# hihixuyang/LQR-Obstacles

Measured on AMD Instinct MI355X. Metric: agent-pair LQR-obstacle evals/sec, higher is better.
Workload: dtype f64

## Files before the change

### lqr-obstacles_amd/csrc/lqro_qhull3.hpp

```cpp
#pragma once
#include "lqro_qhull.hpp"
#include "lqro_lp.hpp"

namespace lqro {

#ifndef Q3_NEWCAP
#define Q3_NEWCAP 128
#endif
#ifndef Q3_VISCAP
#define Q3_VISCAP 192
#endif
#define Q3_MOVCAP 16
#define Q3_HZCAP 24
#define Q3_COPCAP 8
#define Q3_FSTK 512
#define Q3_ND (Q3_NEWCAP + Q3_MOVCAP)
#define Q3_WAVES 4
#define Q3_HR 4
#ifndef Q3_W0_SLEEP
#define Q3_W0_SLEEP 1
#endif
#ifndef Q3_W1_SLEEP
#define Q3_W1_SLEEP 1
#endif
#ifndef Q3_W2_SLEEP
#define Q3_W2_SLEEP 1
#endif
#ifndef Q3_FL
#define Q3_FL 2240
#endif
#define Q3_PROF_RETRY (32 + 2 * 4096 + 16)
#ifdef LQRO_QHULL_PROFILE
#define Q3_CAPBIT(b) (b)
#else
#define Q3_CAPBIT(b) 0
#endif

struct Q3G {
  double pl[4];
  int nb[3];
  int fa;
  unsigned key;
  unsigned cc;
  int pad[2];
};

struct Q3V {
  double p[9];
  double pad;
  int id[4];
};

struct Q3W {
  double* Pr;
  double* Pf;
  Q3G* G;
  Q3V* vv;
  double* ncoord;
  int* soff;
  double* fdist;
  int* sb;
  int* pq;
  int* pdst;
  double* pdd;
  double* ncoord2;
  unsigned* mark2;
  unsigned* ctr;
  unsigned short* hvis;
  int* hcop;
  int* fq;
  unsigned* fqk;
  HullPt* fqc;
  int FC, SB, HNP, QC;
};

__host__ __device__ inline size_t q3_align(size_t b) { return (b + 255) & ~(size_t)255; }

__host__ __device__ inline size_t q3_worker_bytes(int HNP) {
  const size_t FC = 2 * (size_t)HNP + Q3_NEWCAP + 16, SB = (size_t)QH_SBMULT * HNP, QC = 4 * (size_t)HNP + 64;
  const size_t NG = FC > Q3_FL ? FC - Q3_FL : 1;
  return q3_align(24 * (size_t)HNP) * 2 + q3_align(64 * NG) + q3_align(96 * FC) + q3_align(72 * Q3_NEWCAP) +
         q3_align(4 * FC) +
         q3_align(8 * FC) + q3_align(4 * SB) + q3_align(4 * (size_t)HNP) * 2 + q3_align(8 * (size_t)HNP) +
         q3_align(4 * QC) * 2 + q3_align(32 * QC) + q3_align(72 * Q3_NEWCAP) + q3_align(4 * FC) + 256 +
         q3_align(2 * (Q3_WAVES - 1) * Q3_HZCAP * 64) + q3_align(4 * (Q3_WAVES - 1) * Q3_COPCAP * 64);
}

__device__ inline Q3W q3_worker(char* base, int HNP) {
  Q3W W;
  W.HNP = HNP;
  W.FC = 2 * HNP + Q3_NEWCAP + 16;
  W.SB = QH_SBMULT * HNP;
  W.QC = 4 * HNP + 64;
  const size_t NG = W.FC > Q3_FL ? W.FC - Q3_FL : 1;
  char* p = base;
  auto take = [&](size_t bytes) { char* r = p; p += q3_align(bytes); return r; };
  W.Pr = reinterpret_cast<double*>(take(24 * (size_t)HNP));
  W.Pf = reinterpret_cast<double*>(take(24 * (size_t)HNP));
  W.G = reinterpret_cast<Q3G*>(take(64 * NG));
  W.vv = reinterpret_cast<Q3V*>(take(96 * (size_t)W.FC));
  W.ncoord = reinterpret_cast<double*>(take(72 * (size_t)Q3_NEWCAP));
  W.soff = reinterpret_cast<int*>(take(4 * (size_t)W.FC));
  W.fdist = reinterpret_cast<double*>(take(8 * (size_t)W.FC));
  W.sb = reinterpret_cast<int*>(take(4 * (size_t)W.SB));
  W.pq = reinterpret_cast<int*>(take(4 * (size_t)HNP));
  W.pdst = reinterpret_cast<int*>(take(4 * (size_t)HNP));
  W.pdd = reinterpret_cast<double*>(take(8 * (size_t)HNP));
  W.fq = reinterpret_cast<int*>(take(4 * (size_t)W.QC));
  W.fqk = reinterpret_cast<unsigned*>(take(4 * (size_t)W.QC));
  W.fqc = reinterpret_cast<HullPt*>(take(32 * (size_t)W.QC));
  W.ncoord2 = reinterpret_cast<double*>(take(72 * (size_t)Q3_NEWCAP));
  W.mark2 = reinterpret_cast<unsigned*>(take(4 * (size_t)W.FC));
  W.ctr = reinterpret_cast<unsigned*>(take(256));
  W.hvis = reinterpret_cast<unsigned short*>(take(2 * (Q3_WAVES - 1) * Q3_HZCAP * 64));
  W.hcop = reinterpret_cast<int*>(take(4 * (Q3_WAVES - 1) * Q3_COPCAP * 64));
  return W;
}

struct Q3L {
  int n, fail, job, slot;
  double eps;
  double tr[3 * 128];
  double rk[4];
  int ri[4];
  int scan[4];
  double4 pl[Q3_FL];
  ushort4 tp[Q3_FL];
  unsigned key[Q3_FL];
  unsigned cc[Q3_FL];
  unsigned short fstk[Q3_FSTK];
  int visf[Q3_VISCAP];
  int vsoff[Q3_VISCAP], vscnt[Q3_VISCAP], vinc[Q3_VISCAP];
  int vvert[3 * Q3_VISCAP];
  int repl[Q3_VISCAP];
  int nslot[Q3_NEWCAP];
  int nv[3 * Q3_NEWCAP];
  int nhz[Q3_NEWCAP], nhskip[Q3_NEWCAP];
  int nn1[Q3_NEWCAP], nn2[Q3_NEWCAP];
  alignas(32) double npl[4 * Q3_NEWCAP];
  int nflag[Q3_NEWCAP];
  int movf[Q3_MOVCAP];
  int oldf[Q3_MOVCAP];
  int dfac[Q3_ND], dcnt[Q3_ND], doff[Q3_ND], dchamp[Q3_ND], pcnt[Q3_ND];
  double dmax[Q3_ND];
  double dchp[3 * Q3_ND];
  int cop[Q3_COPCAP * 64];
  unsigned short hvis[Q3_HZCAP * 64];
  int sp_visf[Q3_VISCAP];
  int sp_repl[Q3_VISCAP];
  int sp_v1[Q3_NEWCAP], sp_v2[Q3_NEWCAP], sp_nhz[Q3_NEWCAP], sp_nhskip[Q3_NEWCAP], sp_nflag[Q3_NEWCAP];
  int sp_nn1[Q3_NEWCAP], sp_nn2[Q3_NEWCAP];
  int sp_vvert[3 * Q3_VISCAP];
  alignas(32) double sp_npl[4 * Q3_NEWCAP];
  unsigned short mark[Q3_FL];
  unsigned short sp_cand[3 * Q3_VISCAP];
  int sp_hz, sp_hnvis, pf_done, pf_np;
  int pf_vsoff[Q3_VISCAP], pf_vscnt[Q3_VISCAP];
  HullPt pf_pre[64];
  unsigned char pf_prea[64];
  double sp_apex[3];
  double c_dist[8];
  double c_interior[3];
  int ph, sp_done, sp_ok, sp_facet, sp_furthest, sp_pos, sp_nvis, sp_nnew, sp_status, sp_sharp;
  int sp_gdone;
  unsigned sp_key;
  int pub_qhead, pub_qtail;
  int pub_adopt, pub_nnew;
  double hr_d[Q3_HR * 64];
  unsigned short hr_f[Q3_HR * 64];
  unsigned short hr_k[Q3_HR * 64];
  int hr_ls[Q3_HR], hr_st[Q3_HR];
  unsigned hctl;
  int hbusy, hcons;
  unsigned ectl;
  int edone, ej_np, ej_nd, ej_ndnew, ej_init, ej_nvis;
  int hq_end, hq_from, hq_np, hq_sharp, hq_init;
  int hq_findbestnew, hq_notsharp, hq_nnew, hq_nmov, hq_nvis;
  double hq_max_outside;
#ifdef LQRO_QHULL_LONGPROF
  unsigned long long hprof[12];
  unsigned long long lp_pubr, lp_doner;
#endif
  int big_slot;
  int qflags;
#ifdef LQRO_QHULL_PROFILE
  unsigned long long pub_t, done_t, done_t2;
  unsigned long long pub_r, start_r, done_r;
#endif
};
static_assert(sizeof(Q3L) <= 160 * 1024, "k_qhull's LDS exceeds a CU");

struct Q3S {
  int nalloc, nfs, sbtop, status, qhead, qtail;
  int nins;
  unsigned keyc;
  unsigned key0_last;
  int nnew, nvis, nmov, nold;
  int findbestnew, notsharp;
  int hgen;
  int egen;
  double MAXabs_coord, MAXsumcoord, MAXwidth, NEARzero[3];
  double DISTround, MINvisible, MAXcoplanar, MINoutside, MINdenom, MINdenom_2, max_outside;
  double interior[3];
  unsigned long long tph[32];
  unsigned long long tq;
  unsigned long long tw, nw;
  unsigned long long tdl;
  unsigned long long tw1, nw1;
  unsigned long long tse, tsn;
  unsigned long long tfr, nsp;
  unsigned long long tfr2, trel;
  unsigned long long r_start, r_done, r_seen, r_gseen;
  unsigned long long tseen, tpre, npre, tstart;
  int prev1;
  unsigned long long tps[24], nps;
  unsigned long long lp_n, lp_pts, lp_t, lp_all, lp_tloc, lp_wait, lp_adopt, lp_tail, lp_tw;
  unsigned long long lp_own, lp_got, lp_hwait, lp_stop, lp_ev, lp_posts;
};

#if defined(LQRO_QHULL_PROFILE) && defined(LQRO_QHULL_PROF_LIGHT)
#define Q3T(k) do { const unsigned long long t_ = __builtin_amdgcn_s_memtime(); S.tph[k] += t_ - S.tq; S.tq = t_; } while (0)
#elif defined(LQRO_QHULL_PROFILE)
#define Q3T(k) do { __builtin_amdgcn_s_waitcnt(0); const unsigned long long t_ = __builtin_amdgcn_s_memtime(); S.tph[k] += t_ - S.tq; S.tq = t_; } while (0)
#else
#define Q3T(k) do {} while (0)
#endif
#define Q3_PROF_W1 (32 + 2 * 4096 + 48 + 4 * 4096)
#define Q3_PROF_LONG (Q3_PROF_W1 + 64)
struct Q3P {
  unsigned long long tq2 = 0;
  unsigned long long t[16];
  unsigned long long tq;
};
#if defined(LQRO_QHULL_PROFILE) && defined(LQRO_QHULL_PROF_LIGHT)
#define W1T(k) do { const unsigned long long t_ = __builtin_amdgcn_s_memtime(); P.t[k] += t_ - P.tq; P.tq = t_; } while (0)
#elif defined(LQRO_QHULL_PROFILE)
#define W1T(k) do { __builtin_amdgcn_s_waitcnt(0); const unsigned long long t_ = __builtin_amdgcn_s_memtime(); P.t[k] += t_ - P.tq; P.tq = t_; } while (0)
#else
#define W1T(k) do {} while (0)
#endif
#ifdef LQRO_QHULL_PROFILE
#define Q3C(k, v) do { S.tph[k] += (unsigned long long)(v); } while (0)
#else
#define Q3C(k, v) do {} while (0)
#endif

#define Q3_AS3 __attribute__((address_space(3)))
#define Q3_AS1 __attribute__((address_space(1)))
template <class T> __device__ __forceinline__ T q3_lds(const T& r) { return *(const Q3_AS3 T*)(&r); }
template <class T> __device__ __forceinline__ void q3_lds_st(T& r, const T& v) { *(Q3_AS3 T*)(&r) = v; }
template <class T> __device__ __forceinline__ T q3_glb(const T& r) { return *(const Q3_AS1 T*)(&r); }
template <class T> __device__ __forceinline__ void q3_glb_st(T& r, const T& v) { *(Q3_AS1 T*)(&r) = v; }
typedef double q3_v4d __attribute__((ext_vector_type(4)));
typedef int q3_v4i __attribute__((ext_vector_type(4)));
typedef unsigned q3_v2u __attribute__((ext_vector_type(2)));
__device__ __forceinline__ double4 q3_lds(const double4& r) {
  const q3_v4d v = *(const Q3_AS3 q3_v4d*)(&r);
  return make_double4(v.x, v.y, v.z, v.w);
}
__device__ __forceinline__ void q3_lds_st(double4& r, const double4& v) {
  q3_v4d t; t.x = v.x; t.y = v.y; t.z = v.z; t.w = v.w;
  *(Q3_AS3 q3_v4d*)(&r) = t;
}
__device__ __forceinline__ ushort4 q3_lds(const ushort4& r) {
  const q3_v2u v = *(const Q3_AS3 q3_v2u*)(&r);
  return make_ushort4((unsigned short)(v.x & 0xffffu), (unsigned short)(v.x >> 16), (unsigned short)(v.y & 0xffffu),
                      (unsigned short)(v.y >> 16));
}
__device__ __forceinline__ void q3_lds_st(ushort4& r, const ushort4& v) {
  q3_v2u t;
  t.x = (unsigned)v.x | ((unsigned)v.y << 16);
  t.y = (unsigned)v.z | ((unsigned)v.w << 16);
  *(Q3_AS3 q3_v2u*)(&r) = t;
}
__device__ __forceinline__ double4 q3_glb(const double4& r) {
  const q3_v4d v = *(const Q3_AS1 q3_v4d*)(&r);
  return make_double4(v.x, v.y, v.z, v.w);
}
__device__ __forceinline__ void q3_glb_st(double4& r, const double4& v) {
  q3_v4d t; t.x = v.x; t.y = v.y; t.z = v.z; t.w = v.w;
  *(Q3_AS1 q3_v4d*)(&r) = t;
}
__device__ __forceinline__ int4 q3_glb(const int4& r) {
  const q3_v4i v = *(const Q3_AS1 q3_v4i*)(&r);
  return make_int4(v.x, v.y, v.z, v.w);
}
__device__ __forceinline__ void q3_glb_st(int4& r, const int4& v) {
  q3_v4i t; t.x = v.x; t.y = v.y; t.z = v.z; t.w = v.w;
  *(Q3_AS1 q3_v4i*)(&r) = t;
}

struct Q3Col {
  unsigned short* vis;
  int* cop;
};
template <bool G, class T> __device__ __forceinline__ T q3_col(const T& r) {
  if constexpr (G) return q3_glb(r);
  else return q3_lds(r);
}
template <bool G, class T> __device__ __forceinline__ void q3_col_st(T& r, const T& v) {
  if constexpr (G) q3_glb_st(r, v);
  else q3_lds_st(r, v);
}
__device__ __forceinline__ Q3Col q3_col0(const Q3L& L, int lane) {
  Q3Col C;
  C.vis = const_cast<unsigned short*>(L.hvis) + lane;
  C.cop = const_cast<int*>(L.cop) + lane;
  return C;
}
__device__ __forceinline__ Q3Col q3_colh(const Q3W& W, int wave, int lane) {
  Q3Col C;
  C.vis = W.hvis + (size_t)(wave - 1) * Q3_HZCAP * 64 + lane;
  C.cop = W.hcop + (size_t)(wave - 1) * Q3_COPCAP * 64 + lane;
  return C;
}

__device__ __forceinline__ void q3_get(const Q3W& W, const Q3L& L, int f, double* q, int* nb, int* fa) {
  if (f < Q3_FL) {
    const double4 p = q3_lds(L.pl[f]);
    const ushort4 t = q3_lds(L.tp[f]);
    q[0] = p.x; q[1] = p.y; q[2] = p.z; q[3] = p.w;
    nb[0] = t.x; nb[1] = t.y; nb[2] = t.z; *fa = t.w;
  } else {
    const Q3G& g = W.G[f - Q3_FL];
    const double4 p = q3_glb(*reinterpret_cast<const double4*>(g.pl));
    const int4 t = q3_glb(*reinterpret_cast<const int4*>(g.nb));
    q[0] = p.x; q[1] = p.y; q[2] = p.z; q[3] = p.w;
    nb[0] = t.x; nb[1] = t.y; nb[2] = t.z; *fa = t.w;
  }
}
__device__ __forceinline__ void q3_pl(const Q3W& W, const Q3L& L, int f, double* q) {
  const double4 p = f < Q3_FL ? q3_lds(L.pl[f]) : q3_glb(*reinterpret_cast<const double4*>(W.G[f - Q3_FL].pl));
  q[0] = p.x; q[1] = p.y; q[2] = p.z; q[3] = p.w;
}
__device__ __forceinline__ int q3_nb(const Q3W& W, const Q3L& L, int f, int k) {
  if (f < Q3_FL) return q3_lds(reinterpret_cast<const unsigned short*>(&L.tp[f])[k]);
  return q3_glb(W.G[f - Q3_FL].nb[k]);
}
__device__ __forceinline__ void q3_tp(const Q3W& W, const Q3L& L, int f, int* nb, int* fa) {
  if (f < Q3_FL) {
    const ushort4 t = q3_lds(L.tp[f]);
    nb[0] = t.x; nb[1] = t.y; nb[2] = t.z; *fa = t.w;
  } else {
    const int4 t = q3_glb(*reinterpret_cast<const int4*>(W.G[f - Q3_FL].nb));
    nb[0] = t.x; nb[1] = t.y; nb[2] = t.z; *fa = t.w;
  }
}
__device__ __forceinline__ int q3_fa(const Q3W& W, const Q3L& L, int f) {
  return f < Q3_FL ? (int)q3_lds(L.tp[f].w) : q3_glb(W.G[f - Q3_FL].fa);
}
__device__ __forceinline__ unsigned q3_key(const Q3W& W, const Q3L& L, int f) {
  return f < Q3_FL ? q3_lds(L.key[f]) : q3_glb(W.G[f - Q3_FL].key);
}
__device__ __forceinline__ unsigned q3_cc(const Q3W& W, const Q3L& L, int f) {
  return f < Q3_FL ? q3_lds(L.cc[f]) : q3_glb(W.G[f - Q3_FL].cc);
}
__device__ __forceinline__ void q3_set_fa(const Q3W& W, Q3L& L, int f, int fa) {
  if (f < Q3_FL) q3_lds_st(L.tp[f].w, (unsigned short)fa);
  else q3_glb_st(W.G[f - Q3_FL].fa, fa);
}
__device__ __forceinline__ void q3_set_nb(const Q3W& W, Q3L& L, int f, int k, int v) {
  if (f < Q3_FL) q3_lds_st(reinterpret_cast<unsigned short*>(&L.tp[f])[k], (unsigned short)v);
  else q3_glb_st(W.G[f - Q3_FL].nb[k], v);
}
__device__ __forceinline__ void q3_set_key(const Q3W& W, Q3L& L, int f, unsigned k) {
  if (f < Q3_FL) q3_lds_st(L.key[f], k);
  else q3_glb_st(W.G[f - Q3_FL].key, k);
}
__device__ __forceinline__ void q3_set_cc(const Q3W& W, Q3L& L, int f, unsigned c) {
  if (f < Q3_FL) q3_lds_st(L.cc[f], c);
  else q3_glb_st(W.G[f - Q3_FL].cc, c);
}
__device__ __forceinline__ void q3_set_facet(const Q3W& W, Q3L& L, int f, const double* q, int nb0, int nb1, int nb2,
                                             int fa) {
  if (f < Q3_FL) {
    q3_lds_st(L.pl[f], make_double4(q[0], q[1], q[2], q[3]));
    q3_lds_st(L.tp[f], make_ushort4((unsigned short)nb0, (unsigned short)nb1, (unsigned short)nb2, (unsigned short)fa));
  } else {
    Q3G& g = W.G[f - Q3_FL];
    q3_glb_st(*reinterpret_cast<double4*>(g.pl), make_double4(q[0], q[1], q[2], q[3]));
    q3_glb_st(*reinterpret_cast<int4*>(g.nb), make_int4(nb0, nb1, nb2, fa));
  }
}

__device__ __forceinline__ QhS q3_as_qhs(const Q3S& S) {
  QhS T;
  T.DISTround = S.DISTround;
  T.MINdenom = S.MINdenom;
  T.MINdenom_2 = S.MINdenom_2;
  for (int k = 0; k < 3; k++) T.NEARzero[k] = S.NEARzero[k];
  return T;
}

__device__ inline void q3_plane(const Q3S& S, int& status, const double* r0, const double* r1, const double* r2,
                                int top, double* q, bool* flipped) {
  const double dX10 = r1[0] - r0[0], dY10 = r1[1] - r0[1], dZ10 = r1[2] - r0[2];
  const double dX20 = r2[0] - r0[0], dY20 = r2[1] - r0[1], dZ20 = r2[2] - r0[2];
  double n[3];
  n[0] = QH_DET2(dY20, dZ20, dY10, dZ10);
  n[1] = QH_DET2(dX10, dZ10, dX20, dZ20);
  n[2] = QH_DET2(dX20, dY20, dX10, dY10);
  double norm = sqrt(n[0] * n[0] + n[1] * n[1] + n[2] * n[2]);
  if (norm > S.MINdenom) {
    if (!top) norm = -norm;
    n[0] /= norm;
    n[1] /= norm;
    n[2] /= norm;
  } else {
    status |= QHS_SINGULAR;
  }
  double off = -(r0[0] * n[0] + r0[1] * n[1] + r0[2] * n[2]);
  const double d2 = off + (r2[0] * n[0] + r2[1] * n[1] + r2[2] * n[2]);
  const double d1 = off + (r1[0] * n[0] + r1[1] * n[1] + r1[2] * n[2]);
  if (d2 > S.DISTround || d2 < -S.DISTround || d1 > S.DISTround || d1 < -S.DISTround) {
    const QhS T = q3_as_qhs(S);
    qh_plane_gauss(T, status, r0, r1, r2, top, n, &off);
  }
  q[0] = n[0]; q[1] = n[1]; q[2] = n[2]; q[3] = off;
  const double di = off + S.interior[0] * n[0] + S.interior[1] * n[1] + S.interior[2] * n[2];
  *flipped = di >= -S.DISTround;
}

__device__ __forceinline__ double q3_distq(const double* q, const double* p) {
  return q[3] + p[0] * q[0] + p[1] * q[1] + p[2] * q[2];
}

__device__ __forceinline__ int q3_scan_add(int v) {
  v += __builtin_amdgcn_update_dpp(0, v, 0x111, 0xf, 0xf, false);
  v += __builtin_amdgcn_update_dpp(0, v, 0x112, 0xf, 0xf, false);
  v += __builtin_amdgcn_update_dpp(0, v, 0x114, 0xf, 0xf, false);
  v += __builtin_amdgcn_update_dpp(0, v, 0x118, 0xf, 0xf, false);
  v += __builtin_amdgcn_update_dpp(0, v, 0x142, 0xa, 0xf, false);
  v += __builtin_amdgcn_update_dpp(0, v, 0x143, 0xc, 0xf, false);
  return v;
}

#define Q3_MAXSTEP(V, CTRL, RM)                                                                    \
  do {                                                                                           \
    const long long u_ = __double_as_longlong(V);                                                \
    const int lo_ = __builtin_amdgcn_update_dpp(-1, (int)u_, CTRL, RM, 0xf, false);              \
    const int hi_ = __builtin_amdgcn_update_dpp((int)0xFFEFFFFF, (int)(u_ >> 32), CTRL, RM, 0xf, false); \
    V = fmax(V, __longlong_as_double(((long long)hi_ << 32) | (long long)(unsigned)lo_));        \
  } while (0)
__device__ __forceinline__ double q3_scan_max(double v) {
  Q3_MAXSTEP(v, 0x111, 0xf);
  Q3_MAXSTEP(v, 0x112, 0xf);
  Q3_MAXSTEP(v, 0x114, 0xf);
  Q3_MAXSTEP(v, 0x118, 0xf);
  Q3_MAXSTEP(v, 0x142, 0xa);
  Q3_MAXSTEP(v, 0x143, 0xc);
  return v;
}

__device__ __forceinline__ void q3_place(unsigned long long grp, int lane, unsigned long long ltmask,
                                         double dd, const HullPt& pt, int off, int lim, int& cnt, double& mx,
                                         int& champ, double& cx, double& cy, double& cz, int& wpos, int& wr) {
  const bool mem = (grp >> lane) & 1ull;
  const int cb = cnt + __popcll(grp & ltmask);
  double run = -DBL_MAX;
  if (grp & (grp - 1ull)) {
    const double inc = q3_scan_max(mem ? dd : -DBL_MAX);
    const long long u_ = __double_as_longlong(inc);
    const int lo_ = __builtin_amdgcn_update_dpp(-1, (int)u_, 0x138, 0xf, 0xf, false);
    const int hi_ = __builtin_amdgcn_update_dpp((int)0xFFEFFFFF, (int)(u_ >> 32), 0x138, 0xf, 0xf, false);
    run = __longlong_as_double(((long long)hi_ << 32) | (long long)(unsigned)lo_);
  }
  if (cnt > 0) run = fmax(run, mx);
  const bool rec = mem && (cb == 0 || run < dd);
  const unsigned long long recm = __ballot(rec);
  const unsigned long long prevm = recm & ltmask;
  int pq = 0;
  if (recm & (recm - 1ull)) {
    const int pl = prevm ? 63 - __clzll((long long)prevm) : lane;
    pq = __shfl(pt.q, pl);
  }
  if (mem && cb > 0 && off + cb - 1 < lim) {
    wpos = off + cb - 1;
    wr = rec ? (prevm ? pq : champ) : pt.q;
  }
  if (recm) {
    const int l = 63 - __clzll((long long)recm);
    champ = __builtin_amdgcn_readlane(pt.q, l);
    cx = hl_rl(pt.x, l); cy = hl_rl(pt.y, l); cz = hl_rl(pt.z, l);
    mx = hl_rl(dd, l);
  }
  cnt += __popcll(grp);
}

template <bool G>
__device__ inline int q3_findbesthorizon(const Q3W& W, const Q3S& S, const Q3L& L, const double* p, int startfacet,
                                         double* bestdist, int& lstatus, const Q3Col& C) {
  int bestfacet = startfacet;
  const double searchdist = S.max_outside + 2 * S.DISTround + fmax(S.MINvisible, S.MAXcoplanar);
  double minsearch = *bestdist - searchdist;
  unsigned short* vis = C.vis;
  int nvis = 0;
  int* cop = C.cop;
  int ncop = 0;
  int nextfacet = -1, nextnb[3] = {-1, -1, -1};
  q3_col_st<G>(vis[0], (unsigned short)startfacet);
  nvis = 1;
  int cur[3] = {q3_nb(W, L, startfacet, 0), q3_nb(W, L, startfacet, 1), q3_nb(W, L, startfacet, 2)};
  for (;;) {
    double q[3][4];
    int fl[3], nn[3][3];
    for (int k = 0; k < 3; k++) q3_get(W, L, cur[k], q[k], nn[k], &fl[k]);
    bool seen3[3] = {false, false, false};
    for (int t = 0; t < nvis; t++) {
      const int v = q3_col<G>(vis[64 * t]);
      seen3[0] |= v == cur[0]; seen3[1] |= v == cur[1]; seen3[2] |= v == cur[2];
    }
    for (int k = 0; k < 3; k++) {
      const int nb = cur[k];
      const bool seen = seen3[k] || (k >= 1 && nb == cur[0]) || (k == 2 && nb == cur[1]);
      if (seen) continue;
      if (nvis == Q3_HZCAP) { lstatus |= QHS_CAPACITY | Q3_CAPBIT(QHS_CAP_HZ); return bestfacet; }
      q3_col_st<G>(vis[64 * nvis], (unsigned short)nb);
      nvis++;
      if (!(fl[k] & QF_FLIPPED)) {
        const double dist = q3_distq(q[k], p);
        if (dist > *bestdist) {
          minsearch = dist - searchdist;
          if (dist > *bestdist + searchdist) ncop = 0;
          bestfacet = nb;
          *bestdist = dist;
        } else if (dist < minsearch) {
          continue;
        }
      }
      if (nextfacet >= 0) {
        if (ncop == Q3_COPCAP) { lstatus |= QHS_CAPACITY | Q3_CAPBIT(QHS_CAP_COP); return bestfacet; }
        q3_col_st<G>(cop[64 * ncop++], nextfacet);
      }
      nextfacet = nb;
      nextnb[0] = nn[k][0]; nextnb[1] = nn[k][1]; nextnb[2] = nn[k][2];
    }
    if (nextfacet >= 0) {
      nextfacet = -1;
      cur[0] = nextnb[0]; cur[1] = nextnb[1]; cur[2] = nextnb[2];
      continue;
    }
    if (!ncop) break;
    int facet;
    if (ncop == 1) { facet = q3_col<G>(cop[0]); ncop = 0; }
    else facet = q3_col<G>(cop[64 * --ncop]);
    cur[0] = q3_nb(W, L, facet, 0); cur[1] = q3_nb(W, L, facet, 1); cur[2] = q3_nb(W, L, facet, 2);
  }
  return bestfacet;
}

template <bool G>
__device__ inline int q3_findbestnew(const Q3W& W, const Q3S& S, const Q3L& L, const double* p, int s0,
                                     double* dist, int bestoutside, int* isoutside, int& lstatus, const Q3Col& C) {
  double bestdist = -DBL_MAX / 2;
  int bestfacet = -1;
  const double distoutside = fmax(2 * S.MINoutside, S.max_outside);
  *isoutside = 1;
  const int total = S.nnew + S.nmov;
  auto fetch = [&](int t, int& f, int& fl, double* q) {
    if (t < S.nnew - s0 || t >= S.nnew - s0 + S.nmov) {
      const int u = t < S.nnew - s0 ? s0 + t : t - (S.nnew - s0) - S.nmov;
      f = L.nslot[u];
      const double4 v = q3_lds(*reinterpret_cast<const double4*>(L.npl + 4 * u));
      q[0] = v.x; q[1] = v.y; q[2] = v.z; q[3] = v.w;
      fl = L.nflag[u];
    } else {
      f = L.movf[t - (S.nnew - s0)];
      q3_pl(W, L, f, q);
      fl = q3_fa(W, L, f);
    }
  };
  for (int t0 = 0; t0 < total; t0 += 4) {
    int f[4], fl[4];
    double q[4][4];
#pragma unroll
    for (int k = 0; k < 4; k++) {
      f[k] = -1; fl[k] = QF_FLIPPED;
      if (t0 + k < total) fetch(t0 + k, f[k], fl[k], q[k]);
    }
#pragma unroll
    for (int k = 0; k < 4; k++) {
      if (fl[k] & QF_FLIPPED) continue;
      const double d = q3_distq(q[k], p);
      if (d > bestdist) {
        bestfacet = f[k];
        if (!bestoutside && d >= distoutside) { *dist = d; return bestfacet; }
        bestdist = d;
      }
    }
  }
  bestfacet = q3_findbesthorizon<G>(W, S, L, p, bestfacet >= 0 ? bestfacet : L.nslot[s0], &bestdist, lstatus, C);
  *dist = bestdist;
  if (bestdist < S.MINoutside) *isoutside = 0;
  return bestfacet;
}

__device__ inline int q3_sharpnewfacets(const Q3S& S, const Q3L& L, int lane) {
  if (S.nnew == 0) return 0;
  const bool q0 = L.npl[0] > 0, q1 = L.npl[1] > 0, q2 = L.npl[2] > 0;
  bool diff = false;
  for (int t = lane; t < S.nnew; t += 64) {
    const double* n = L.npl + 4 * t;
    diff |= (n[0] > 0) != q0 || (n[1] > 0) != q1 || (n[2] > 0) != q2;
  }
  return __ballot(diff) != 0ull;
}

template <bool G>
__device__ inline int q3_locate(const Q3W& W, const Q3S& S, const Q3L& L, const double* p, int s0, int sharp,
                                double* bestdist_out, int* isoutside, int* trigger, int& lstatus, const Q3Col& C) {
  *trigger = 0;
  if (sharp == 2) return q3_findbestnew<G>(W, S, L, p, s0, bestdist_out, 1, isoutside, lstatus, C);
  if (S.findbestnew) return q3_findbestnew<G>(W, S, L, p, s0, bestdist_out, 0, isoutside, lstatus, C);
  double bestdist = -DBL_MAX / 2;
  int bestu = -1;
  *isoutside = 1;
  unsigned long long m0 = 0ull, m1 = 0ull;
  if (!(L.nflag[s0] & QF_FLIPPED)) {
    const double d = q3_distq(L.npl + 4 * s0, p);
    if (d >= S.MINoutside) { *bestdist_out = d; return L.nslot[s0]; }
    bestdist = d;
    bestu = s0;
  }
  if (s0 < 64) m0 |= 1ull << s0; else m1 |= 1ull << (s0 - 64);
  int u = s0;
  while (u >= 0) {
    int nxt = -1;
    const int cand[2] = {L.nn1[u], L.nn2[u]};
    const int cfl[2] = {L.nflag[cand[0]], L.nflag[cand[1]]};
    double cq[2][4];
#pragma unroll
    for (int k = 0; k < 2; k++) {
      const double4 v = q3_lds(*reinterpret_cast<const double4*>(L.npl + 4 * cand[k]));
      cq[k][0] = v.x; cq[k][1] = v.y; cq[k][2] = v.z; cq[k][3] = v.w;
    }
#pragma unroll
    for (int k = 0; k < 2; k++) {
      const int c = cand[k];
      const bool was = c < 64 ? (m0 >> c) & 1ull : (m1 >> (c - 64)) & 1ull;
      if (was) continue;
      if (c < 64) m0 |= 1ull << c; else m1 |= 1ull << (c - 64);
      if (!(cfl[k] & QF_FLIPPED)) {
        const double d = q3_distq(cq[k], p);
        if (d > bestdist) {
          if (d >= S.MINoutside) { *bestdist_out = d; return L.nslot[c]; }
          bestu = c;
          bestdist = d;
          nxt = c;
          break;
        }
      }
    }
    u = nxt;
  }
  if (bestu < 0) return q3_findbestnew<G>(W, S, L, p, 0, bestdist_out, 0, isoutside, lstatus, C);
  if (!S.notsharp && bestdist < -S.DISTround) {
    *trigger = 1;
    if (sharp) return q3_findbestnew<G>(W, S, L, p, bestu, bestdist_out, 0, isoutside, lstatus, C);
  }
  const int bf = q3_findbesthorizon<G>(W, S, L, p, L.nslot[bestu], &bestdist, lstatus, C);
  *bestdist_out = bestdist;
  if (bestdist < S.MINoutside) *isoutside = 0;
  return bf;
}

__device__ __forceinline__ bool q3_in_movf(const Q3S& S, const Q3L& L, int f) {
  for (int t = 0; t < S.nmov; t++)
    if (L.movf[t] == f) return true;
  return false;
}

__device__ __forceinline__ HullPt q3_seqpt(const Q3W& W, const Q3L& L, int nvis, bool init, int pos, int* start) {
  HullPt r;
  if (init) {
    const int q = W.pq[pos];
    r.x = W.Pr[3 * (size_t)q]; r.y = W.Pr[3 * (size_t)q + 1]; r.z = W.Pr[3 * (size_t)q + 2];
    r.q = q;
    r.pad = 0;
    *start = 0;
    return r;
  }
  int a = 0, b = nvis - 1;
  while (a < b) {
    const int mid = (a + b) >> 1;
    if (L.vinc[mid] > pos) b = mid;
    else a = mid + 1;
  }
  *start = L.repl[a] >= 0 ? L.repl[a] : 0;
  const int q = W.sb[L.vsoff[a] + pos - (L.vinc[a] - L.vscnt[a])];
  r.x = W.Pr[3 * (size_t)q]; r.y = W.Pr[3 * (size_t)q + 1]; r.z = W.Pr[3 * (size_t)q + 2];
  r.q = q;
  r.pad = 0;
  return r;
}

__device__ __forceinline__ int q3_ld_acq(const int* p) {
  return __hip_atomic_load(p, __ATOMIC_ACQUIRE, __HIP_MEMORY_SCOPE_WORKGROUP);
}
__device__ __forceinline__ void q3_st_rel(int* p, int v) {
  __hip_atomic_store(p, v, __ATOMIC_RELEASE, __HIP_MEMORY_SCOPE_WORKGROUP);
}
__device__ __forceinline__ void q3_st_rel_lds(int* p, int v) {
  __builtin_amdgcn_fence(__ATOMIC_RELEASE, "workgroup", "local");
  __hip_atomic_store(p, v, __ATOMIC_RELAXED, __HIP_MEMORY_SCOPE_WORKGROUP);
}
__device__ __forceinline__ int q3_wait(const int* p, int v, bool ne) {
  int x = q3_ld_acq(p);
  for (long w = 0; (ne ? x == v : x != v) && w < (1l << 24); ++w) {
    __builtin_amdgcn_s_sleep(Q3_W0_SLEEP);
    x = q3_ld_acq(p);
  }
  return x;
}

template <bool G>
__device__ __forceinline__ void q3_chunk_locate(const Q3W& W, const Q3S& S, const Q3L& L, int c, int from, int np,
                                                int sharp, bool init, int lane, const HullPt& pre, int prestart,
                                                int prec, HullPt& pt, int& f, double& d, int& isout, int& trig,
                                                int& ls, const Q3Col& C) {
  const int pos = c + lane;
  pt = pre;
  f = -1; d = 0.0; isout = 0; trig = 0;
  if (pos >= from && pos < np) {
    int start = prestart;
    if (c != prec) pt = q3_seqpt(W, L, S.nvis, init, pos, &start);
    const double p[3] = {pt.x, pt.y, pt.z};
    f = q3_locate<G>(W, S, L, p, start, sharp, &d, &isout, &trig, ls, C);
  }
}

__device__ inline bool q3_help(const Q3W& W, Q3L& L, int lane, const Q3Col& C) {
  const unsigned v = (unsigned)q3_ld_acq(reinterpret_cast<const int*>(&L.hctl));
  if (v == 0u) return false;
  const int k = (int)(v & 0xffffu);
  if (k >= L.hq_end || k >= hl_ld(&L.hcons) + Q3_HR) return false;
  int got = 0;
  if (lane == 0) {
    __hip_atomic_fetch_add(&L.hbusy, 1, __ATOMIC_SEQ_CST, __HIP_MEMORY_SCOPE_WORKGROUP);
    unsigned e = v;
    got = __hip_atomic_compare_exchange_strong(&L.hctl, &e, v + 1u, __ATOMIC_SEQ_CST, __ATOMIC_SEQ_CST,
                                               __HIP_MEMORY_SCOPE_WORKGROUP);
    if (!got) __hip_atomic_fetch_add(&L.hbusy, -1, __ATOMIC_SEQ_CST, __HIP_MEMORY_SCOPE_WORKGROUP);
  }
  if (!__builtin_amdgcn_readfirstlane(got)) return false;
#ifdef LQRO_QHULL_LONGPROF
  const unsigned long long th0 = __builtin_amdgcn_s_memrealtime();
#endif
  Q3S S;
  S.MINvisible = L.c_dist[0]; S.MAXcoplanar = L.c_dist[1]; S.DISTround = L.c_dist[2];
  S.MINoutside = 2 * S.MINvisible;
  S.findbestnew = L.hq_findbestnew; S.notsharp = L.hq_notsharp;
  S.nnew = L.hq_nnew; S.nmov = L.hq_nmov; S.nvis = L.hq_nvis;
  S.max_outside = L.hq_max_outside;
  HullPt pt, pre;
  pre.x = pre.y = pre.z = 0.0; pre.q = -1; pre.pad = 0;
  int f, isout, trig, ls = 0;
  double d;
  const int from = L.hq_from, np = L.hq_np, pos = 64 * k + lane;
  q3_chunk_locate<true>(W, S, L, 64 * k, from, np, L.hq_sharp, L.hq_init != 0, lane, pre, 0, -1, pt, f, d, isout,
                        trig, ls, C);
#ifdef LQRO_QHULL_LONGPROF
  const unsigned long long th1 = __builtin_amdgcn_s_memrealtime();
#endif
  int kind = 0, dst = -1, dfa = 0;
  if (pos >= from && pos < np) {
    if (isout) {
      dst = f;
      dfa = q3_fa(W, L, f);
      if (!(dfa & QF_NEW) && (q3_cc(W, L, f) & 0xffffu) == 0 && !q3_in_movf(S, L, f)) kind |= 4;
    } else if (d >= -S.MAXcoplanar && d > S.max_outside) {
      kind |= 2;
    }
    if (trig) kind |= 1;
  }
  const bool old = dst >= 0 && !(dfa & QF_NEW);
  const int b = k % Q3_HR;
  L.hr_d[64 * b + lane] = d;
  L.hr_f[64 * b + lane] = (unsigned short)dst;
  L.hr_k[64 * b + lane] = (unsigned short)(kind | (old ? 8 : 0) | ((dst >= 0 && !old ? (dfa >> 8) + 1 : 0) << 8));
  const int st = qh_wave_or(ls);
  if (lane == 0) {
    L.hr_ls[b] = st;
    q3_st_rel_lds(&L.hr_st[b], k + 1);
    __hip_atomic_fetch_add(&L.hbusy, -1, __ATOMIC_SEQ_CST, __HIP_MEMORY_SCOPE_WORKGROUP);
#ifdef LQRO_QHULL_LONGPROF
    const unsigned long long th2 = __builtin_amdgcn_s_memrealtime();
    atomicAdd(&L.hprof[0], 1ull);
    atomicAdd(&L.hprof[1], th1 - th0);
    atomicAdd(&L.hprof[2], th2 - th0);
#endif
  }
  return true;
}

__device__ inline void q3_locate_seq(const Q3W& W, Q3S& S, Q3L& L, int np, int sharp, bool init, int lane,
                                     const HullPt& pre, int prestart, bool havepre, int& rg, double& rd,
                                     HullPt& rpt) {
  for (int t = lane; t < Q3_NEWCAP; t += 64) L.pcnt[t] = 0;
  S.nold = 0;
  rg = -1;
  rd = 0.0;
  rpt = pre;
  hl_sync();
  const bool help = np > 64 && (L.qflags & 1);
  const Q3Col C0 = q3_col0(L, lane);
  auto post = [&](int from2) {
    S.hgen = S.hgen % 32767 + 1;
    if (lane == 0) {
      L.hq_end = (np + 63) >> 6; L.hq_from = from2; L.hq_np = np; L.hq_sharp = sharp; L.hq_init = init ? 1 : 0;
      L.hq_findbestnew = S.findbestnew; L.hq_notsharp = S.notsharp; L.hq_nnew = S.nnew; L.hq_nmov = S.nmov;
      L.hq_nvis = S.nvis; L.hq_max_outside = S.max_outside;
      L.hcons = from2 >> 6;
      for (int b = 0; b < Q3_HR; b++) L.hr_st[b] = 0;
      q3_st_rel(reinterpret_cast<int*>(&L.hctl), (int)(((unsigned)S.hgen << 16) | (unsigned)((from2 >> 6) + 1)));
    }
  };
  auto stop = [&]() {
    if (lane == 0) __hip_atomic_exchange(&L.hctl, 0u, __ATOMIC_SEQ_CST, __HIP_MEMORY_SCOPE_WORKGROUP);
    int b = __hip_atomic_load(&L.hbusy, __ATOMIC_SEQ_CST, __HIP_MEMORY_SCOPE_WORKGROUP);
    for (long w = 0; b != 0 && w < (1l << 24); ++w) {
      __builtin_amdgcn_s_sleep(Q3_W0_SLEEP);
      b = __hip_atomic_load(&L.hbusy, __ATOMIC_SEQ_CST, __HIP_MEMORY_SCOPE_WORKGROUP);
    }
    if (b != 0) S.status |= QHS_CAPACITY | QHS_TIMEOUT;
  };
  int from = 0;
  while (from < np && !(S.status & QHS_CAPACITY)) {
    int ev_pos = np, ev_kind = 0, ev_dst = -1;
    double ev_d = 0.0;
    if (help) post(from);
    bool first = help;
    for (int c = from & ~63; c < np; c += 64) {
      Q3C(23, 1);
      const int pos = c + lane;
      const bool act = pos >= from && pos < np;
      int kind = 0, ls = 0, dst = -1, dfa = 0;
      double d = 0.0;
      HullPt pt = pre;
      int f = -1, isout = 0, trig = 0;
      bool mine = !help || first;
      if (help && !first) {
        const int k = c >> 6, b = k % Q3_HR;
        int st = q3_ld_acq(&L.hr_st[b]);
        if (st != k + 1) {
          int m = 0;
          if (lane == 0) {
            unsigned e = __hip_atomic_load(&L.hctl, __ATOMIC_RELAXED, __HIP_MEMORY_SCOPE_WORKGROUP);
            if ((e & 0xffffu) == (unsigned)k)
              m = __hip_atomic_compare_exchange_strong(&L.hctl, &e, e + 1u, __ATOMIC_RELAXED, __ATOMIC_RELAXED,
                                                       __HIP_MEMORY_SCOPE_WORKGROUP);
          }
          mine = __builtin_amdgcn_readfirstlane(m) != 0;
#ifdef LQRO_QHULL_LONGPROF
          const unsigned long long tw0 = __builtin_amdgcn_s_memrealtime();
#endif
          if (!mine) st = q3_wait(&L.hr_st[b], k + 1, false);
#ifdef LQRO_QHULL_LONGPROF
          if (!mine) S.lp_hwait += __builtin_amdgcn_s_memrealtime() - tw0;
#endif
        }
#ifdef LQRO_QHULL_LONGPROF
        if (mine) S.lp_own++; else S.lp_got++;
#endif
        int kv = 0;
        if (!mine) {
          if (st != k + 1) { S.status |= QHS_CAPACITY | QHS_TIMEOUT; break; }
          const int fv = L.hr_f[64 * b + lane];
          kv = L.hr_k[64 * b + lane];
          ls = L.hr_ls[b];
          dst = fv == 0xffff ? -1 : fv;
          kind = act ? kv & 7 : 0;
          dfa = (kv & 8) ? 0 : (((kv >> 8) - 1) << 8) | QF_NEW;
          d = L.hr_d[64 * b + lane];
        }
      }
      first = false;
      Q3T(12);
      if (mine) q3_chunk_locate<false>(W, S, L, c, from, np, sharp, init, lane, pre, prestart, havepre ? 0 : -1, pt, f,
                                       d, isout, trig, ls, C0);
      Q3T(13);
      if (mine && act) {
        if (isout) {
          dst = f;
          dfa = q3_fa(W, L, f);
          if (!(dfa & QF_NEW) && (q3_cc(W, L, f) & 0xffffu) == 0 && !q3_in_movf(S, L, f)) kind |= 4;
        } else if (d >= -S.MAXcoplanar && d > S.max_outside) {
          kind |= 2;
        }
        if (trig) kind |= 1;
      }
      S.status |= qh_wave_or(ls);
      if (help && lane == 0) q3_st_rel_lds(&L.hcons, (c >> 6) + 1);
      const unsigned long long b = __ballot(kind != 0);
      const int last = b ? __ffsll((long long)b) - 1 : 63;
      const bool fin = act && lane <= last;
      int g = -1;
      if (fin && dst >= 0 && (dfa & QF_NEW)) {
        g = dfa >> 8;
        atomicAdd(&L.pcnt[g], 1);
      }
      unsigned long long old = __ballot(fin && dst >= 0 && !(dfa & QF_NEW));
      while (old) {
        const int l = __ffsll((long long)old) - 1;
        old &= old - 1;
        const int f = __builtin_amdgcn_readlane(dst, l);
        int k = -1;
        for (int t = 0; t < S.nold; t++)
          if (L.oldf[t] == f) k = t;
        if (k < 0) {
          if (S.nold == Q3_MOVCAP) { S.status |= QHS_CAPACITY | Q3_CAPBIT(QHS_CAP_MOV); continue; }
          k = S.nold++;
          if (lane == 0) { L.oldf[k] = f; L.pcnt[Q3_NEWCAP + k] = 0; L.dfac[Q3_NEWCAP + k] = f; }
          hl_sync();
        }
        if (lane == 0) L.pcnt[Q3_NEWCAP + k]++;
        if (lane == l) g = Q3_NEWCAP + k;
        hl_sync();
      }
      if (fin) {
        rg = g;
        rd = d;
        rpt = pt;
        if (np > 64) {
          W.pdst[pos] = g;
          W.pdd[pos] = d;
        }
      }
      hl_sync();
      Q3T(14);
      if (b) {
        ev_pos = c + last;
        ev_kind = __builtin_amdgcn_readlane(kind, last);
        ev_dst = __builtin_amdgcn_readlane(dst, last);
        ev_d = hl_rl(d, last);
        break;
      }
    }
#ifdef LQRO_QHULL_LONGPROF
    const unsigned long long ts0 = __builtin_amdgcn_s_memrealtime();
#endif
    if (help) stop();
#ifdef LQRO_QHULL_LONGPROF
    if (help) { S.lp_stop += __builtin_amdgcn_s_memrealtime() - ts0; S.lp_posts++; if (ev_pos < np) S.lp_ev++; }
#endif
    if (S.status & QHS_CAPACITY) return;
    if (ev_pos < np) {
      Q3C(24, 1);
      if (ev_kind & 1) {
        if (sharp) S.findbestnew = 1;
        else S.notsharp = 1;
      }
      if (ev_kind & 2) S.max_outside = ev_d;
      if (ev_kind & 4) {
        const int f = ev_dst;
        if (S.nmov == Q3_MOVCAP) {
          S.status |= QHS_CAPACITY | Q3_CAPBIT(QHS_CAP_MOV);
          return;
        }
        if (lane == 0) {
          L.movf[S.nmov] = f;
          if (init) {
            int t0 = 0;
            for (int t = 0; t < S.nnew; t++)
              if (L.nslot[t] == f) t0 = t;
            for (int t = t0; t + 1 < S.nnew; t++) {
              L.nslot[t] = L.nslot[t + 1];
              for (int k = 0; k < 4; k++) L.npl[4 * t + k] = L.npl[4 * (t + 1) + k];
              L.nflag[t] = L.nflag[t + 1];
            }
            double q[4];
            q3_pl(W, L, f, q);
            L.nslot[S.nnew - 1] = f;
            for (int k = 0; k < 4; k++) L.npl[4 * (S.nnew - 1) + k] = q[k];
            L.nflag[S.nnew - 1] = q3_fa(W, L, f);
          }
        }
        q3_set_key(W, L, f, S.keyc);
        S.keyc++;
        S.nmov++;
      }
      hl_sync();
    }
    from = ev_pos + 1;
  }
}

__device__ inline void q3_emit_bucket(const Q3W& W, Q3L& L, int lane, int b) {
  const int np = L.ej_np, nd = L.ej_nd, ndnew = L.ej_ndnew, nvis = L.ej_nvis;
  const bool init = L.ej_init != 0;
  const int gl = lane < ndnew ? lane : Q3_NEWCAP + (lane - ndnew);
  const bool has = lane < nd && (lane & 3) == b && L.pcnt[gl];
  int Rc = 0, Rch = -1, Ro = 0;
  double Rm = 0.0, Rx = 0.0, Ry = 0.0, Rz = 0.0;
  if (has) {
    Rc = L.dcnt[gl]; Rm = L.dmax[gl]; Rch = L.dchamp[gl]; Ro = L.doff[gl];
    Rx = L.dchp[3 * gl]; Ry = L.dchp[3 * gl + 1]; Rz = L.dchp[3 * gl + 2];
  }
  const unsigned long long ltmask = (1ull << lane) - 1ull;
  int ng = -1;
  double ndd = 0.0;
  HullPt npt;
  npt.x = npt.y = npt.z = 0.0; npt.q = -1; npt.pad = 0;
  auto ldc = [&](int c) {
    const int pos = c + lane;
    ng = -1;
    ndd = 0.0;
    if (pos < np) {
      ng = W.pdst[pos];
      ndd = W.pdd[pos];
      int st;
      npt = q3_seqpt(W, L, nvis, init, pos, &st);
    }
  };
  ldc(0);
  for (int c = 0; c < np; c += 64) {
    const int g = ng;
    const double dd = ndd;
    const HullPt pt = npt;
    if (c + 64 < np) ldc(c + 64);
    const int i = g < 0 ? -1 : (g < Q3_NEWCAP ? g : ndnew + (g - Q3_NEWCAP));
    const bool mine = i >= 0 && (i & 3) == b;
    unsigned long long todo = __ballot(mine);
    int wpos = -1, wr = 0;
    while (todo) {
      const int lead = __ffsll((long long)todo) - 1;
      const int gg = __builtin_amdgcn_readlane(g, lead);
      const unsigned long long grp = __ballot(mine && g == gg);
      todo &= ~grp;
      const int l = __builtin_amdgcn_readlane(i, lead);
      int cnt = __builtin_amdgcn_readlane(Rc, l), champ = __builtin_amdgcn_readlane(Rch, l);
      double mx = hl_rl(Rm, l), cx = hl_rl(Rx, l), cy = hl_rl(Ry, l), cz = hl_rl(Rz, l);
      q3_place(grp, lane, ltmask, dd, pt, __builtin_amdgcn_readlane(Ro, l), W.SB, cnt, mx, champ, cx, cy, cz, wpos,
               wr);
      if (lane == l) { Rc = cnt; Rm = mx; Rch = champ; Rx = cx; Ry = cy; Rz = cz; }
    }
    if (wpos >= 0) W.sb[wpos] = wr;
  }
  if (has) {
    L.dcnt[gl] = Rc; L.dmax[gl] = Rm; L.dchamp[gl] = Rch;
    L.dchp[3 * gl] = Rx; L.dchp[3 * gl + 1] = Ry; L.dchp[3 * gl + 2] = Rz;
  }
}

__device__ __forceinline__ int q3_emit_claim(Q3L& L, int lane) {
  int k = -1;
  if (lane == 0) {
    for (;;) {
      unsigned v = (unsigned)q3_ld_acq(reinterpret_cast<const int*>(&L.ectl));
      if (v == 0u || (v & 0xffu) >= 4u) break;
      unsigned e = v;
      if (__hip_atomic_compare_exchange_strong(&L.ectl, &e, v + 1u, __ATOMIC_ACQ_REL, __ATOMIC_RELAXED,
                                               __HIP_MEMORY_SCOPE_WORKGROUP)) {
        k = (int)(v & 0xffu);
        break;
      }
    }
  }
  return __builtin_amdgcn_readfirstlane(k);
}

__device__ inline bool q3_emit_help(const Q3W& W, Q3L& L, int lane) {
  const unsigned v = (unsigned)q3_ld_acq(reinterpret_cast<const int*>(&L.ectl));
  if (v == 0u || (v & 0xffu) >= 4u) return false;
  const int k = q3_emit_claim(L, lane);
  if (k < 0) return false;
  q3_emit_bucket(W, L, lane, k);
  if (lane == 0) {
    __builtin_amdgcn_fence(__ATOMIC_RELEASE, "workgroup");
    __hip_atomic_fetch_add(&L.edone, 1, __ATOMIC_RELEASE, __HIP_MEMORY_SCOPE_WORKGROUP);
  }
  return true;
}

__device__ inline void q3_emit_seq(const Q3W& W, Q3S& S, Q3L& L, int np, int ndnew, bool init, int lane, int rg,
                                   double rd, const HullPt& rpt) {
  if (S.status & QHS_CAPACITY) return;
  if (!init && np <= 64 && S.nold == 0 && ndnew <= 64) {
    const int g = lane;
    int pc = 0, f = 0;
    if (g < ndnew) { f = L.nslot[g]; pc = L.pcnt[g]; }
    const int inc = q3_scan_add(pc);
    const int top = S.sbtop + __builtin_amdgcn_readlane(inc, 63);
    if (top > W.SB) {
      S.status |= QHS_CAPACITY | Q3_CAPBIT(QHS_CAP_SB);
      return;
    }
    const int doff = S.sbtop + inc - pc;
    S.sbtop = top;
    Q3T(15);
    int dcnt = 0, dchamp = -1;
    double dmax = 0.0, dx = 0.0, dy = 0.0, dz = 0.0;
    const unsigned long long ltmask = (1ull << lane) - 1ull;
    const int rgl = lane < np ? rg : -1;
    unsigned long long todo = __ballot(rgl >= 0);
    int wpos = -1, wr = 0;
    Q3T(16);
    while (todo) {
      const int lead = __ffsll((long long)todo) - 1;
      const int gg = __builtin_amdgcn_readlane(rgl, lead);
      const unsigned long long grp = __ballot(rgl == gg);
      todo &= ~grp;
      int cnt = 0, champ = -1;
      double mx = 0.0, cx = 0.0, cy = 0.0, cz = 0.0;
      q3_place(grp, lane, ltmask, rd, rpt, __builtin_amdgcn_readlane(doff, gg), W.SB, cnt, mx, champ, cx, cy, cz,
               wpos, wr);
      Q3C(25, 1);
      if (lane == gg) { dcnt = cnt; dmax = mx; dchamp = champ; dx = cx; dy = cy; dz = cz; }
    }
    if (wpos >= 0) W.sb[wpos] = wr;
    Q3T(17);
    if (g < ndnew && pc) {
      W.sb[doff + dcnt - 1] = dchamp;
      W.soff[f] = doff;
      W.fdist[f] = dmax;
      q3_set_cc(W, L, f, (unsigned)dcnt | ((unsigned)dchamp << 16));
    }
    const bool has = g < ndnew && pc > 0;
    const unsigned long long b = __ballot(has);
    int qt = S.qtail;
    if (has) {
      const int at = qt + __popcll(b & ltmask);
      if (at < W.QC) {
        W.fq[at] = f;
        W.fqk[at] = S.key0_last + (unsigned)g;
        HullPt r;
        r.x = dx; r.y = dy; r.z = dz; r.q = dchamp; r.pad = 0;
        W.fqc[at] = r;
      }
    }
    qt += __popcll(b);
    if (qt > W.QC) S.status |= QHS_CAPACITY | Q3_CAPBIT(QHS_CAP_FACETS);
    S.qtail = qt;
    hl_sync();
    Q3T(18);
    return;
  }
  const int nd = ndnew + S.nold;
  int base = S.sbtop;
  for (int c0 = 0; c0 < nd; c0 += 64) {
    const int i = c0 + lane;
    int size = 0, g = -1, cnt0 = 0;
    if (i < nd) {
      g = i < ndnew ? i : Q3_NEWCAP + (i - ndnew);
      if (g < Q3_NEWCAP) L.dfac[g] = L.nslot[g];
      if (L.pcnt[g]) {
        cnt0 = g < Q3_NEWCAP ? 0 : (int)(q3_cc(W, L, L.dfac[g]) & 0xffffu);
        size = cnt0 + L.pcnt[g];
      }
    }
    const int inc = q3_scan_add(size);
    if (size) {
      L.doff[g] = base + inc - size;
      L.dcnt[g] = cnt0;
      L.dmax[g] = 0.0;
      L.dchamp[g] = -1;
    }
    base += __builtin_amdgcn_readlane(inc, 63);
  }
  if (base > W.SB) {
    S.status |= QHS_CAPACITY | Q3_CAPBIT(QHS_CAP_SB);
    return;
  }
  S.sbtop = base;
  hl_sync();
  for (int k = 0; k < S.nold; k++) {
    const int g = Q3_NEWCAP + k;
    const int f = L.dfac[g];
    const int cnt0 = L.dcnt[g];
    if (!L.pcnt[g] || !cnt0) continue;
    const int off0 = W.soff[f];
    const int off = L.doff[g];
    for (int t = lane; t < cnt0 - 1; t += 64) W.sb[off + t] = W.sb[off0 + t];
    const int chq = W.sb[off0 + cnt0 - 1];
    const double fd = W.fdist[f];
    if (lane == 0) {
      L.dchamp[g] = chq;
      L.dchp[3 * g] = W.Pr[3 * (size_t)chq]; L.dchp[3 * g + 1] = W.Pr[3 * (size_t)chq + 1];
      L.dchp[3 * g + 2] = W.Pr[3 * (size_t)chq + 2];
      L.dmax[g] = fd;
    }
    hl_sync();
  }
  hl_sync();
  Q3T(15);
  if (np > 64 && nd <= 64 && (L.qflags & 16)) {
    S.egen = S.egen % 0xffffff + 1;
    if (lane == 0) {
      L.ej_np = np; L.ej_nd = nd; L.ej_ndnew = ndnew; L.ej_init = init ? 1 : 0; L.ej_nvis = S.nvis;
      L.edone = 0;
      q3_st_rel(reinterpret_cast<int*>(&L.ectl), (int)((unsigned)S.egen << 8));
    }
    int mine = 0;
    for (int k = q3_emit_claim(L, lane); k >= 0; k = q3_emit_claim(L, lane)) {
      q3_emit_bucket(W, L, lane, k);
      ++mine;
    }
    hl_sync();
    int dn = q3_ld_acq(&L.edone);
    for (long w = 0; dn != 4 - mine && w < (1l << 24); ++w) {
      __builtin_amdgcn_s_sleep(Q3_W0_SLEEP);
      dn = q3_ld_acq(&L.edone);
    }
    if (lane == 0) __hip_atomic_store(&L.ectl, 0u, __ATOMIC_RELAXED, __HIP_MEMORY_SCOPE_WORKGROUP);
    if (dn != 4 - mine) { S.status |= QHS_CAPACITY | QHS_TIMEOUT; return; }
  } else {
  const bool inl = nd <= 64 && (L.qflags & 2);
  int Rc = 0, Rch = -1, Ro = 0;
  double Rm = 0.0, Rx = 0.0, Ry = 0.0, Rz = 0.0;
  if (inl && lane < nd) {
    const int g = lane < ndnew ? lane : Q3_NEWCAP + (lane - ndnew);
    if (L.pcnt[g]) {
      Rc = L.dcnt[g]; Rm = L.dmax[g]; Rch = L.dchamp[g]; Ro = L.doff[g];
      Rx = L.dchp[3 * g]; Ry = L.dchp[3 * g + 1]; Rz = L.dchp[3 * g + 2];
    }
  }
  int ng = -1;
  double ndd = 0.0;
  HullPt npt = rpt;
  auto ldc = [&](int c) {
    const int pos = c + lane;
    ng = -1;
    ndd = 0.0;
    if (pos < np) {
      ng = W.pdst[pos];
      ndd = W.pdd[pos];
      int st;
      npt = q3_seqpt(W, L, S.nvis, init, pos, &st);
    }
  };
  if (np > 64) ldc(0);
  for (int c = 0; c < np; c += 64) {
    const int pos = c + lane;
    const bool act = pos < np;
    int g = rg;
    double dd = rd;
    HullPt pt = rpt;
    if (np > 64) {
      g = ng;
      dd = ndd;
      pt = npt;
      if (c + 64 < np) ldc(c + 64);
    } else if (!act) {
      g = -1;
    }
    Q3T(16);
    unsigned long long todo = __ballot(g >= 0);
    const unsigned long long ltmask = (1ull << lane) - 1ull;
    int wpos = -1, wr = 0;
    while (todo) {
      const int lead = __ffsll((long long)todo) - 1;
      const int gg = __builtin_amdgcn_readlane(g, lead);
      const unsigned long long grp = __ballot(g == gg);
      todo &= ~grp;
      if (inl) {
        const int l = gg < Q3_NEWCAP ? gg : ndnew + (gg - Q3_NEWCAP);
        int cnt = __builtin_amdgcn_readlane(Rc, l), champ = __builtin_amdgcn_readlane(Rch, l);
        double mx = hl_rl(Rm, l), cx = hl_rl(Rx, l), cy = hl_rl(Ry, l), cz = hl_rl(Rz, l);
        q3_place(grp, lane, ltmask, dd, pt, __builtin_amdgcn_readlane(Ro, l), W.SB, cnt, mx, champ, cx, cy, cz, wpos,
                 wr);
        if (lane == l) { Rc = cnt; Rm = mx; Rch = champ; Rx = cx; Ry = cy; Rz = cz; }
      } else {
        int cnt = L.dcnt[gg];
        double mx = L.dmax[gg];
        int champ = L.dchamp[gg];
        double cx = L.dchp[3 * gg], cy = L.dchp[3 * gg + 1], cz = L.dchp[3 * gg + 2];
        const int off = L.doff[gg];
        q3_place(grp, lane, ltmask, dd, pt, off, W.SB, cnt, mx, champ, cx, cy, cz, wpos, wr);
        if (lane == 0) {
          L.dcnt[gg] = cnt; L.dmax[gg] = mx; L.dchamp[gg] = champ;
          L.dchp[3 * gg] = cx; L.dchp[3 * gg + 1] = cy; L.dchp[3 * gg + 2] = cz;
        }
        hl_sync();
      }
      Q3C(25, 1);
    }
    if (wpos >= 0) W.sb[wpos] = wr;
  }
  if (inl && lane < nd) {
    const int g = lane < ndnew ? lane : Q3_NEWCAP + (lane - ndnew);
    if (L.pcnt[g]) {
      L.dcnt[g] = Rc; L.dmax[g] = Rm; L.dchamp[g] = Rch;
      L.dchp[3 * g] = Rx; L.dchp[3 * g + 1] = Ry; L.dchp[3 * g + 2] = Rz;
    }
  }
  }
  hl_sync();
  Q3T(17);
  for (int i = lane; i < nd; i += 64) {
    const int g = i < ndnew ? i : Q3_NEWCAP + (i - ndnew);
    if (!L.pcnt[g]) continue;
    const int f = L.dfac[g];
    W.sb[L.doff[g] + L.dcnt[g] - 1] = L.dchamp[g];
    W.soff[f] = L.doff[g];
    W.fdist[f] = L.dmax[g];
    q3_set_cc(W, L, f, (unsigned)L.dcnt[g] | ((unsigned)L.dchamp[g] << 16));
  }
  hl_sync();
  if (init) return;
  int qt = S.qtail;
  for (int c = 0; c < ndnew; c += 64) {
    const int t = c + lane;
    const bool has = t < ndnew && L.pcnt[t] > 0;
    const unsigned long long b = __ballot(has);
    if (has) {
      const int at = qt + __popcll(b & ((1ull << lane) - 1ull));
      if (at < W.QC) {
        W.fq[at] = L.nslot[t];
        W.fqk[at] = q3_key(W, L, L.nslot[t]);
        HullPt r;
        r.x = L.dchp[3 * t]; r.y = L.dchp[3 * t + 1]; r.z = L.dchp[3 * t + 2]; r.q = L.dchamp[t]; r.pad = 0;
        W.fqc[at] = r;
      }
    }
    qt += __popcll(b);
  }
  for (int t = lane; t < S.nmov; t += 64)
    if (qt + t < W.QC) {
      W.fq[qt + t] = L.movf[t];
      W.fqk[qt + t] = q3_key(W, L, L.movf[t]);
      HullPt r;
      r.x = r.y = r.z = 0.0; r.q = -1; r.pad = 0;
      W.fqc[qt + t] = r;
    }
  qt += S.nmov;
  if (qt > W.QC) S.status |= QHS_CAPACITY | Q3_CAPBIT(QHS_CAP_FACETS);
  S.qtail = qt;
  hl_sync();
  Q3T(18);
}

__device__ __forceinline__ int q3_alloc(const Q3S& S, const Q3L& L, int t) {
  if (t < S.nvis) return L.visf[t];
  const int e = t - S.nvis;
  if (e < S.nfs) return L.fstk[S.nfs - 1 - e];
  return S.nalloc + (e - S.nfs);
}

struct Q3QC {
  int qcb, qcn, qf, qp;
  unsigned qk;
  double qx, qy, qz;
  int one, rt;
  double r[6];
  int pc_from, pc_pos, pc_end, pc_f, pc_p;
  unsigned pc_k;
  double pc_x, pc_y, pc_z;
};

__device__ inline void q3_spec(const Q3W& W, Q3L& L, int lane, unsigned short ep, unsigned ep2, Q3QC& Q, Q3P& P,
                               int phase) {
  const unsigned long long ltmask = (1ull << lane) - 1ull;
  Q3S C;
  C.MINvisible = L.c_dist[0]; C.MAXcoplanar = L.c_dist[1]; C.DISTround = L.c_dist[2];
  C.MINdenom = L.c_dist[3]; C.MINdenom_2 = L.c_dist[4];
  for (int k = 0; k < 3; k++) { C.NEARzero[k] = L.c_dist[5 + k]; C.interior[k] = L.c_interior[k]; }
  auto marked = [&](int f) -> bool {
    return f < Q3_FL ? q3_lds(L.mark[f]) == ep : q3_glb(W.mark2[f]) == ep2;
  };
  auto mark = [&](int f) {
    if (f < Q3_FL) q3_lds_st(L.mark[f], ep);
    else q3_glb_st(W.mark2[f], ep2);
  };
  if (L.pub_adopt) {
    const int nn = L.pub_nnew;
    if (Q.one) {
      if (Q.rt >= 0) {
        const int t = Q.rt;
        Q3V& v = W.vv[L.nslot[t]];
        *reinterpret_cast<double4*>(v.p) = make_double4(L.sp_apex[0], L.sp_apex[1], L.sp_apex[2], Q.r[0]);
        *reinterpret_cast<double4*>(v.p + 4) = make_double4(Q.r[1], Q.r[2], Q.r[3], Q.r[4]);
        *reinterpret_cast<double2*>(v.p + 8) = make_double2(Q.r[5], 0.0);
        *reinterpret_cast<int4*>(v.id) = make_int4(L.nv[3 * t], L.nv[3 * t + 1], L.nv[3 * t + 2], 0);
      }
    } else {
      for (int t = lane; t < nn; t += 64) {
        Q3V& v = W.vv[L.nslot[t]];
        const double* nc = W.ncoord2 + 9 * t;
        *reinterpret_cast<double4*>(v.p) = make_double4(L.sp_apex[0], L.sp_apex[1], L.sp_apex[2], nc[0]);
        *reinterpret_cast<double4*>(v.p + 4) = make_double4(nc[1], nc[2], nc[3], nc[4]);
        *reinterpret_cast<double2*>(v.p + 8) = make_double2(nc[5], 0.0);
        *reinterpret_cast<int4*>(v.id) = make_int4(L.nv[3 * t], L.nv[3 * t + 1], L.nv[3 * t + 2], 0);
      }
    }
  }
  Q.one = 0;
  Q.rt = -1;
  W1T(1);
#ifdef LQRO_QHULL_LONGPROF
  const unsigned long long tq0_ = __builtin_amdgcn_s_memrealtime();
  int reloads_ = 0;
#endif
  int ok = 0;
  const int qt = L.pub_qtail;
  int facet = -1, furthest = -1, fpos = -1;
  unsigned fkey = 0;
  double apex[3] = {0.0, 0.0, 0.0};
  int qh0 = L.pub_qhead;
  if (Q.pc_from >= 0 && Q.pc_from == qh0 && L.pub_adopt) {
    if (Q.pc_pos >= 0) {
      const int fa = q3_fa(W, L, Q.pc_f);
      const unsigned c = q3_cc(W, L, Q.pc_f);
      if ((fa & QF_LIVE) && !(fa & QF_VISIBLE) && q3_key(W, L, Q.pc_f) == Q.pc_k && (c & 0xffffu) > 0) {
        fpos = Q.pc_pos;
        facet = Q.pc_f;
        fkey = Q.pc_k;
        furthest = (int)(c >> 16);
        if (Q.pc_p == furthest) {
          apex[0] = Q.pc_x; apex[1] = Q.pc_y; apex[2] = Q.pc_z;
        } else {
          apex[0] = W.Pr[3 * (size_t)furthest];
          apex[1] = W.Pr[3 * (size_t)furthest + 1];
          apex[2] = W.Pr[3 * (size_t)furthest + 2];
        }
      } else {
        qh0 = Q.pc_pos + 1;
      }
    } else {
      qh0 = max(qh0, Q.pc_end);
    }
  }
  Q.pc_from = -1;
  for (int qh = qh0; facet < 0 && qh < qt;) {
    if (qh >= Q.qcb + Q.qcn || qh < Q.qcb) {
#ifdef LQRO_QHULL_LONGPROF
      ++reloads_;
#endif
      Q.qcb = qh;
      Q.qcn = min(64, qt - qh);
      if (lane < Q.qcn) {
        Q.qf = W.fq[qh + lane];
        Q.qk = W.fqk[qh + lane];
        const HullPt e = W.fqc[qh + lane];
        Q.qx = e.x; Q.qy = e.y; Q.qz = e.z; Q.qp = e.q;
      }
    }
    bool good = false;
    unsigned c = 0;
    if (lane < Q.qcn && Q.qcb + lane >= qh && Q.qcb + lane < qt) {
      const int fa = q3_fa(W, L, Q.qf);
      c = q3_cc(W, L, Q.qf);
      good = (fa & QF_LIVE) && !(fa & QF_VISIBLE) && q3_key(W, L, Q.qf) == Q.qk && (c & 0xffffu) > 0;
    }
    const unsigned long long b = __ballot(good);
    if (b) {
      const int l = __ffsll((long long)b) - 1;
      fpos = Q.qcb + l;
      facet = __builtin_amdgcn_readlane(Q.qf, l);
      fkey = (unsigned)__builtin_amdgcn_readlane((int)Q.qk, l);
      furthest = (int)((unsigned)__builtin_amdgcn_readlane((int)c, l) >> 16);
      if (__builtin_amdgcn_readlane(Q.qp, l) == furthest) {
        apex[0] = hl_rl(Q.qx, l); apex[1] = hl_rl(Q.qy, l); apex[2] = hl_rl(Q.qz, l);
      } else {
        apex[0] = W.Pr[3 * (size_t)furthest];
        apex[1] = W.Pr[3 * (size_t)furthest + 1];
        apex[2] = W.Pr[3 * (size_t)furthest + 2];
      }
      break;
    }
    qh = Q.qcb + Q.qcn;
  }
  int ls = 0, nvis = 0, nnew = 0, ts = 0, lm = 0;
  W1T(2);
#ifdef LQRO_QHULL_LONGPROF
  const unsigned long long tq1_ = __builtin_amdgcn_s_memrealtime();
  if (lane == 0) { L.hprof[8] += (unsigned long long)reloads_; L.hprof[9] += tq1_ - tq0_; }
#endif
  if (facet >= 0) {
    if (lane == 0) L.sp_visf[0] = facet;
    if (lane < 3) L.sp_cand[lane] = (unsigned short)q3_nb(W, L, facet, lane);
    mark(facet);
    hl_sync();
    nvis = 1;
    bool cap = false;
    for (int lo = 0; lo < nvis && !cap;) {
      const int hi = nvis;
      const int ncand = 3 * (hi - lo);
      for (int c0 = 0; c0 < ncand; c0 += 64) {
        const int c = c0 + lane;
        int nb = -1;
        bool cand = false;
        double q[4] = {0.0, 0.0, 0.0, 0.0};
        int nn[3] = {0, 0, 0};
        if (c < ncand) {
          nb = L.sp_cand[3 * lo + c];
          int fa;
          q3_get(W, L, nb, q, nn, &fa);
          cand = !marked(nb);
        }
        const double dist = cand ? q3_distq(q, apex) : 0.0;
        bool vis = cand && dist >= C.MINvisible;
        if (cand && !vis && dist >= -C.MAXcoplanar) ls |= QHS_COPLANAR;
        bool dup = false;
        for (unsigned long long mm = __ballot(vis); mm;) {
          const int l = __ffsll((long long)mm) - 1;
          mm &= mm - 1;
          dup |= (l < lane) && __builtin_amdgcn_readlane(nb, l) == nb;
        }
        vis = vis && !dup;
        const unsigned long long bv = __ballot(vis);
        if (vis) {
          const int at = nvis + __popcll(bv & ltmask);
          if (at < Q3_VISCAP) {
            L.sp_visf[at] = nb;
            L.sp_cand[3 * at] = (unsigned short)nn[0];
            L.sp_cand[3 * at + 1] = (unsigned short)nn[1];
            L.sp_cand[3 * at + 2] = (unsigned short)nn[2];
          }
          mark(nb);
        }
        nvis += __popcll(bv);
        hl_sync();
      }
      lo = hi;
      if (nvis > Q3_VISCAP) cap = true;
#ifdef LQRO_QHULL_PROFILE
      P.t[11] += 1;
#endif
    }
#ifdef LQRO_QHULL_LONGPROF
    if (lane == 0) L.hprof[10] += __builtin_amdgcn_s_memrealtime() - tq1_;
#endif
    if (!cap && lane == 0) {
      L.sp_hnvis = nvis;
      q3_st_rel_lds(&L.sp_hz, phase);
    }
    W1T(3);
    const bool one = 3 * nvis <= 64;
    int my_t = -1, rv1 = -1, rv2 = -1, mn1 = 0, mn2 = 0;
    double P1[3] = {0.0, 0.0, 0.0}, P2[3] = {0.0, 0.0, 0.0}, PO[3] = {0.0, 0.0, 0.0};
    double Q4[4] = {0.0, 0.0, 0.0, 0.0};
    unsigned long long rb = 0ull;
    if (!cap) {
      for (int vi = lane; vi < nvis; vi += 64) L.sp_repl[vi] = -1;
      hl_sync();
      for (int c0 = 0; c0 < 3 * nvis; c0 += 64) {
        const int c = c0 + lane;
        int vis = -1, nb = -1, hfa = 0;
        bool ridge = false;
        int hn[3] = {-1, -1, -1};
        if (c < 3 * nvis) {
          const int vi = c / 3;
          vis = L.sp_visf[vi];
          nb = L.sp_cand[c];
          q3_tp(W, L, nb, hn, &hfa);
          ridge = !marked(nb);
          if (c == 3 * vi) {
            const Q3V& vw = W.vv[vis];
            L.sp_vvert[3 * vi] = vw.id[0]; L.sp_vvert[3 * vi + 1] = vw.id[1]; L.sp_vvert[3 * vi + 2] = vw.id[2];
          }
        }
        const unsigned long long b = __ballot(ridge);
        if (one) rb = b;
        if (ridge) {
          const int t = nnew + __popcll(b & ltmask);
          const int hskip = hn[0] == vis ? 0 : hn[1] == vis ? 1 : hn[2] == vis ? 2 : -1;
          if (hskip < 0) {
            ts |= QHS_TOPOLOGY;
          } else if (t < Q3_NEWCAP) {
            const Q3V& h = W.vv[nb];
            const int top = (hfa & QF_TOP) ? (hskip & 1) : ((hskip & 1) ^ 1);
            const int i1 = hskip == 0 ? 1 : 0, i2 = hskip == 2 ? 1 : 2;
            double p1[3], p2[3], po[3];
            for (int k = 0; k < 3; k++) {
              p1[k] = h.p[3 * i1 + k];
              p2[k] = h.p[3 * i2 + k];
              po[k] = h.p[3 * hskip + k];
            }
            L.sp_v1[t] = h.id[i1];
            L.sp_v2[t] = h.id[i2];
            L.sp_nhz[t] = nb;
            L.sp_nhskip[t] = hskip;
            atomicMax(&L.sp_repl[c / 3], t);
            double q[4];
            bool flipped;
            int fl = QF_NEW | QF_LIVE | (top ? QF_TOP : 0);
            q3_plane(C, lm, apex, p1, p2, top, q, &flipped);
            if (flipped) { fl |= QF_FLIPPED; lm |= QHS_FLIPPED; }
            L.sp_nflag[t] = fl;
            L.sp_npl[4 * t] = q[0]; L.sp_npl[4 * t + 1] = q[1]; L.sp_npl[4 * t + 2] = q[2]; L.sp_npl[4 * t + 3] = q[3];
            if (one) {
              my_t = t;
              rv1 = h.id[i1];
              rv2 = h.id[i2];
              for (int k = 0; k < 4; k++) Q4[k] = q[k];
              for (int k = 0; k < 3; k++) { P1[k] = p1[k]; P2[k] = p2[k]; PO[k] = po[k]; }
            } else {
              for (int k = 0; k < 3; k++) {
                W.ncoord2[9 * t + k] = p1[k]; W.ncoord2[9 * t + 3 + k] = p2[k]; W.ncoord2[9 * t + 6 + k] = po[k];
              }
            }
          }
        }
        nnew += __popcll(b);
      }
      ok = nnew <= Q3_NEWCAP;
      if (one) {
        Q.one = 1;
        Q.rt = my_t;
        for (int k = 0; k < 3; k++) { Q.r[k] = P1[k]; Q.r[3 + k] = P2[k]; }
      }
      W1T(4);
      if (ok) {
        hl_sync();
        if (one) {
          int nbu[2] = {-1, -1}, cnt[2] = {0, 0};
          int u = 0;
          for (unsigned long long bb = rb; bb; bb &= bb - 1ull, ++u) {
            const int l = __ffsll((long long)bb) - 1;
            const int a = __builtin_amdgcn_readlane(rv1, l), c2 = __builtin_amdgcn_readlane(rv2, l);
            const bool o = u != my_t;
            if (o && (a == rv2 || c2 == rv2)) { nbu[0] = u; cnt[0]++; }
            if (o && (a == rv1 || c2 == rv1)) { nbu[1] = u; cnt[1]++; }
          }
          if (my_t >= 0) {
            if (cnt[0] != 1 || cnt[1] != 1) lm |= QHS_TOPOLOGY;
            mn1 = nbu[0] >= 0 ? nbu[0] : 0;
            mn2 = nbu[1] >= 0 ? nbu[1] : 0;
            L.sp_nn1[my_t] = mn1;
            L.sp_nn2[my_t] = mn2;
          }
        } else {
          for (int t = lane; t < nnew; t += 64) {
            int nbu[2] = {-1, -1}, cnt[2] = {0, 0};
            const int w0 = L.sp_v2[t], w1 = L.sp_v1[t];
#pragma unroll 4
            for (int u = 0; u < nnew; u++) {
              const int a = L.sp_v1[u], bb = L.sp_v2[u];
              const bool o = u != t;
              if (o && (a == w0 || bb == w0)) { nbu[0] = u; cnt[0]++; }
              if (o && (a == w1 || bb == w1)) { nbu[1] = u; cnt[1]++; }
            }
            if (cnt[0] != 1 || cnt[1] != 1) lm |= QHS_TOPOLOGY;
            L.sp_nn1[t] = nbu[0] >= 0 ? nbu[0] : 0;
            L.sp_nn2[t] = nbu[1] >= 0 ? nbu[1] : 0;
          }
        }
        hl_sync();
        W1T(12);
        if (!(qh_wave_or(lm) & QHS_FLIPPED)) {
          auto zero = [&](int t, const double* p1, const double* p2, const double* po) {
            const double d1 = q3_distq(L.sp_npl + 4 * L.sp_nn1[t], p1);
            const double d2 = q3_distq(L.sp_npl + 4 * L.sp_nn2[t], p2);
            const double d3 = q3_distq(L.sp_npl + 4 * t, po);
            if (d1 >= -2 * C.DISTround || d2 >= -2 * C.DISTround || d3 >= -2 * C.DISTround) lm |= QHS_NONCONVEX;
          };
          if (one) {
            if (my_t >= 0) {
              const double4 a = q3_lds(*reinterpret_cast<const double4*>(L.sp_npl + 4 * mn1));
              const double4 b = q3_lds(*reinterpret_cast<const double4*>(L.sp_npl + 4 * mn2));
              const double qa[4] = {a.x, a.y, a.z, a.w}, qb[4] = {b.x, b.y, b.z, b.w};
              const double d1 = q3_distq(qa, P1), d2 = q3_distq(qb, P2), d3 = q3_distq(Q4, PO);
              if (d1 >= -2 * C.DISTround || d2 >= -2 * C.DISTround || d3 >= -2 * C.DISTround) lm |= QHS_NONCONVEX;
            }
          } else {
            for (int t = lane; t < nnew; t += 64) {
              double p1[3], p2[3], po[3];
              for (int k = 0; k < 3; k++) {
                p1[k] = W.ncoord2[9 * t + k]; p2[k] = W.ncoord2[9 * t + 3 + k]; po[k] = W.ncoord2[9 * t + 6 + k];
              }
              zero(t, p1, p2, po);
            }
          }
        }
        W1T(13);
        bool diff = false;
        if (one && rb) {
          const int l0 = __ffsll((long long)rb) - 1;
          const bool q0 = hl_rl(Q4[0], l0) > 0, q1 = hl_rl(Q4[1], l0) > 0, q2 = hl_rl(Q4[2], l0) > 0;
          if (my_t >= 0) diff = (Q4[0] > 0) != q0 || (Q4[1] > 0) != q1 || (Q4[2] > 0) != q2;
        } else if (nnew > 0) {
          const bool q0 = L.sp_npl[0] > 0, q1 = L.sp_npl[1] > 0, q2 = L.sp_npl[2] > 0;
          for (int t = lane; t < nnew; t += 64) {
            const double* nn = L.sp_npl + 4 * t;
            diff |= (nn[0] > 0) != q0 || (nn[1] > 0) != q1 || (nn[2] > 0) != q2;
          }
        }
        const bool sh = __ballot(diff) != 0ull;
        if (lane == 0) L.sp_sharp = sh;
      }
    }
  }
  const int st = qh_wave_or(ls | ts | lm);
  W1T(5);
  hl_sync();
  Q.pc_end = qt;
  if (lane == 0) {
    L.sp_ok = ok;
    L.sp_facet = facet;
    L.sp_key = fkey;
    L.sp_furthest = furthest;
    L.sp_pos = fpos;
    L.sp_nvis = nvis;
    L.sp_nnew = nnew;
    L.sp_status = st;
    L.sp_apex[0] = apex[0]; L.sp_apex[1] = apex[1]; L.sp_apex[2] = apex[2];
  }
}

__device__ inline void q3_prescan(const Q3W& W, Q3L& L, int lane, unsigned short ep, unsigned ep2, Q3QC& Q) {
  Q.pc_from = -1;
  const int from = L.sp_pos, qt = Q.pc_end;
  if (!L.sp_ok || L.sp_facet < 0 || from < 0) return;
  auto marked = [&](int f) -> bool {
    return f < Q3_FL ? q3_lds(L.mark[f]) == ep : q3_glb(W.mark2[f]) == ep2;
  };
  Q.pc_pos = -1;
  for (int qh = from; qh < qt;) {
    if (qh >= Q.qcb + Q.qcn || qh < Q.qcb) {
      Q.qcb = qh;
      Q.qcn = min(64, qt - qh);
      if (lane < Q.qcn) {
        Q.qf = W.fq[qh + lane];
        Q.qk = W.fqk[qh + lane];
        const HullPt e = W.fqc[qh + lane];
        Q.qx = e.x; Q.qy = e.y; Q.qz = e.z; Q.qp = e.q;
      }
    }
    bool good = false;
    if (lane < Q.qcn && Q.qcb + lane >= qh && Q.qcb + lane < qt) {
      const int fa = q3_fa(W, L, Q.qf);
      const unsigned c = q3_cc(W, L, Q.qf);
      good = (fa & QF_LIVE) && !marked(Q.qf) && q3_key(W, L, Q.qf) == Q.qk && (c & 0xffffu) > 0;
    }
    const unsigned long long b = __ballot(good);
    if (b) {
      const int l = __ffsll((long long)b) - 1;
      Q.pc_pos = Q.qcb + l;
      Q.pc_f = __builtin_amdgcn_readlane(Q.qf, l);
      Q.pc_k = (unsigned)__builtin_amdgcn_readlane((int)Q.qk, l);
      Q.pc_p = __builtin_amdgcn_readlane(Q.qp, l);
      Q.pc_x = hl_rl(Q.qx, l); Q.pc_y = hl_rl(Q.qy, l); Q.pc_z = hl_rl(Q.qz, l);
      break;
    }
    qh = Q.qcb + Q.qcn;
  }
  Q.pc_from = from;
}

__device__ inline void q3_prefetch(const Q3W& W, Q3L& L, int lane, int p) {
  const int nvis = L.sp_hnvis;
  int np = 0;
  for (int c0 = 0; c0 < nvis; c0 += 64) {
    const int vi = c0 + lane;
    int cnt = 0;
    if (vi < nvis) {
      const int f = L.sp_visf[vi];
      cnt = (int)(q3_cc(W, L, f) & 0xffffu) - (vi == 0 ? 1 : 0);
      L.pf_vsoff[vi] = W.soff[f];
      L.pf_vscnt[vi] = cnt;
    }
    np += __builtin_amdgcn_readlane(q3_scan_add(cnt), 63);
  }
  hl_sync();
  if (lane < np) {
    int a = 0, base = 0;
    for (;;) {
      const int k = L.pf_vscnt[a];
      if (lane < base + k || a == nvis - 1) break;
      base += k;
      ++a;
    }
    const int q = W.sb[L.pf_vsoff[a] + lane - base];
    HullPt r;
    r.x = W.Pr[3 * (size_t)q]; r.y = W.Pr[3 * (size_t)q + 1]; r.z = W.Pr[3 * (size_t)q + 2];
    r.q = q;
    r.pad = 0;
    L.pf_pre[lane] = r;
    L.pf_prea[lane] = (unsigned char)a;
  }
  hl_sync();
  if (lane == 0) {
    L.pf_np = np;
    q3_st_rel(&L.pf_done, p);
  }
}

__device__ inline void q3_build(const Q3W& W, Q3S& S, Q3L& L, int n, int lane) {
#ifdef LQRO_QHULL_PROFILE
  S.tq = __builtin_amdgcn_s_memtime();
#endif
  const unsigned long long ltmask = (1ull << lane) - 1ull;
  S.status = 0;
  S.nalloc = 1;
  S.nfs = 0;
  S.sbtop = 0;
  S.nnew = S.nvis = S.nmov = S.nold = 0;
  S.findbestnew = S.notsharp = 0;
  S.hgen = 0;
  S.egen = 0;
  S.keyc = 1;
  S.key0_last = 0;
  S.qhead = S.qtail = 0;
  if (W.FC > 65535) {
    S.status |= QHS_CAPACITY | Q3_CAPBIT(QHS_CAP_FACETS);
    return;
  }
  int maxpoints[6];
  S.max_outside = 0.0;
  S.MAXabs_coord = 0.0;
  S.MAXwidth = -DBL_MAX;
  S.MAXsumcoord = 0.0;
  for (int k = 0; k < 3; k++) {
    int mn, mx;
    qh_extreme(W.Pr, n, k, false, lane, &mn);
    qh_extreme(W.Pr, n, k, true, lane, &mx);
    const double maxk = W.Pr[3 * (size_t)mx + k], mink = W.Pr[3 * (size_t)mn + k];
    const double maxcoord = fmax(maxk, -mink);
    const double temp = maxk - mink;
    if (temp > S.MAXwidth) S.MAXwidth = temp;
    if (maxcoord > S.MAXabs_coord) S.MAXabs_coord = maxcoord;
    S.MAXsumcoord += maxcoord;
    maxpoints[2 * k] = mn;
    maxpoints[2 * k + 1] = mx;
    S.NEARzero[k] = 80 * S.MAXsumcoord * DBL_EPSILON;
  }
  {
    double maxdistsum = sqrt(3.0) * S.MAXabs_coord;
    if (S.MAXsumcoord < maxdistsum) maxdistsum = S.MAXsumcoord;
    S.DISTround = DBL_EPSILON * (3 * maxdistsum * 1.01 + S.MAXabs_coord);
    const double MINdenom_1 = fmax(1.0 / DBL_MAX, DBL_MIN);
    S.MINdenom = MINdenom_1 * S.MAXabs_coord;
    S.MINdenom_2 = sqrt(MINdenom_1 * 3) * S.MAXabs_coord;
    S.MINvisible = 0.0 + 2 * S.DISTround;
    S.MAXcoplanar = S.MINvisible;
    S.MINoutside = 2 * S.MINvisible;
  }
  int simplex[4];
  {
    const QhS T = q3_as_qhs(S);
    double maxcoord = -DBL_MAX, mincoord = DBL_MAX;
    int minx = -1, maxx = -1;
    for (int i = 0; i < 6; i++) {
      const double c = W.Pr[3 * (size_t)maxpoints[i]];
      if (maxcoord < c) { maxcoord = c; maxx = maxpoints[i]; }
      if (mincoord > c) { mincoord = c; minx = maxpoints[i]; }
    }
    double maxdet = maxcoord - mincoord;
    int ns = 0;
    simplex[ns++] = minx;
    if (maxx != minx) simplex[ns++] = maxx;
    if (ns < 2) { S.status |= QHS_INPUT; return; }
    for (int i = 2; i < 4; i++) {
      const double prevdet = maxdet;
      int maxpoint = -1, maxnearzero = 0, nearzero;
      maxdet = -1.0;
      for (int m = 0; m < 6; m++) {
        const int p = maxpoints[m];
        bool ins = false;
        for (int t = 0; t < i; t++) ins |= simplex[t] == p;
        if (!ins && p != maxpoint) {
          const double det = fabs(qh_detsimplex(T, W.Pr, simplex, i, p, &nearzero));
          if (det > maxdet) { maxdet = det; maxpoint = p; maxnearzero = nearzero; }
        }
      }
      const double targetdet = prevdet * S.MAXwidth;
      const bool falsenarrow = maxdet > 0.0 && maxdet / targetdet < 1.0e-3;
      if (maxpoint < 0 || maxnearzero || falsenarrow) {
        double key = -1.0;
        int idx = 0x7fffffff;
        for (int q = lane; q < n; q += 64) {
          bool skip = false;
          for (int t = 0; t < 6; t++) skip |= maxpoints[t] == q;
          for (int t = 0; t < i; t++) skip |= simplex[t] == q;
          if (skip) continue;
          const double det = fabs(qh_detsimplex(T, W.Pr, simplex, i, q, &nearzero));
          if (det > key || (det == key && q < idx)) { key = det; idx = q; }
        }
        for (int off = 32; off >= 1; off >>= 1) {
          const double ok = __shfl_xor(key, off);
          const int oi = __shfl_xor(idx, off);
          if (ok > key || (ok == key && oi < idx)) { key = ok; idx = oi; }
        }
        if (idx != 0x7fffffff && key > maxdet) { maxdet = key; maxpoint = idx; }
      }
      if (maxpoint < 0) { S.status |= QHS_INPUT; return; }
      simplex[i] = maxpoint;
    }
  }
  const int pset[4] = {simplex[3], simplex[2], simplex[1], simplex[0]};
  int fs[4];
  {
    int top = 1, tops[4];
    for (int i = 0; i < 4; i++) {
      fs[i] = S.nalloc++;
      tops[i] = top;
      top ^= 1;
    }
    for (int k = 0; k < 3; k++) {
      double c = 0.0;
      for (int t = 0; t < 4; t++) c += W.Pr[3 * (size_t)pset[t] + k];
      S.interior[k] = c / 4;
    }
    int fv[4][3];
    for (int i = 0; i < 4; i++) {
      int m = 0;
      for (int t = 0; t < 4; t++)
        if (t != i) fv[i][m++] = pset[t];
    }
    int ls = 0;
    double q[4][4];
    bool fl[4];
    q3_plane(S, ls, W.Pr + 3 * (size_t)fv[0][0], W.Pr + 3 * (size_t)fv[0][1], W.Pr + 3 * (size_t)fv[0][2], tops[0],
             q[0], &fl[0]);
    if (q3_distq(q[0], S.interior) > S.DISTround)
      for (int i = 0; i < 4; i++) tops[i] ^= 1;
    bool anyflip = false;
    for (int i = 0; i < 4; i++) {
      q3_plane(S, ls, W.Pr + 3 * (size_t)fv[i][0], W.Pr + 3 * (size_t)fv[i][1], W.Pr + 3 * (size_t)fv[i][2],
               tops[i], q[i], &fl[i]);
      anyflip |= fl[i];
    }
    if (anyflip) ls |= QHS_FLIPPED;
    int nbs[4][3];
    for (int i = 0; i < 4; i++) {
      int m = 0;
      for (int t = 0; t < 4; t++)
        if (t != i) nbs[i][m++] = fs[t];
    }
    double minangle = DBL_MAX;
    for (int i = 0; i < 4; i++)
      for (int t = 0; t < 3; t++) {
        int j = 0;
        for (int u = 0; u < 4; u++)
          if (fs[u] == nbs[i][t]) j = u;
        double angle = 0.0;
        for (int k = 0; k < 3; k++) angle += q[i][k] * q[j][k];
        if (angle < minangle) minangle = angle;
      }
    if (minangle < -0.99999999) ls |= QHS_NARROW;
    S.status |= ls;
    hl_sync();
    if (lane == 0)
      for (int i = 0; i < 4; i++) {
        const int f = fs[i];
        q3_set_facet(W, L, f, q[i], nbs[i][0], nbs[i][1], nbs[i][2],
                     QF_LIVE | (tops[i] ? QF_TOP : 0) | (fl[i] ? QF_FLIPPED : 0));
        q3_set_key(W, L, f, S.keyc + i);
        q3_set_cc(W, L, f, 0u);
        Q3V& v = W.vv[f];
        for (int t = 0; t < 3; t++) {
          for (int k = 0; k < 3; k++) v.p[3 * t + k] = W.Pr[3 * (size_t)fv[i][t] + k];
          v.id[t] = fv[i][t];
        }
      }
    S.keyc += 4;
    hl_sync();
    int np = 0;
    for (int c = 0; c < n; c += 64) {
      const int qi = c + lane;
      const bool ok = qi < n && qi != simplex[0] && qi != simplex[1] && qi != simplex[2] && qi != simplex[3];
      const unsigned long long b = __ballot(ok);
      if (ok) W.pq[np + __popcll(b & ltmask)] = qi;
      np += __popcll(b);
    }
    hl_sync();
    const double distoutside = fmax(2 * S.MINoutside, S.max_outside);
    for (int i = 0; i < 4; i++) {
      const int f = fs[i];
      int cnt = 0;
      const int off = S.sbtop;
      double mx = 0.0, cx = 0.0, cy = 0.0, cz = 0.0;
      int champ = -1, w = 0;
      for (int c = 0; c < np; c += 64) {
        const int pos = c + lane;
        HullPt pt;
        pt.x = pt.y = pt.z = 0.0;
        pt.q = -1;
        pt.pad = 0;
        double d = -DBL_MAX;
        if (pos < np) {
          pt.q = W.pq[pos];
          pt.x = W.Pr[3 * (size_t)pt.q]; pt.y = W.Pr[3 * (size_t)pt.q + 1]; pt.z = W.Pr[3 * (size_t)pt.q + 2];
          const double p[3] = {pt.x, pt.y, pt.z};
          d = q3_distq(q[i], p);
        }
        const bool out = pos < np && d >= distoutside;
        const bool keep = pos < np && !out;
        const unsigned long long bk = __ballot(keep);
        hl_sync();
        if (keep) W.pq[w + __popcll(bk & ltmask)] = pt.q;
        w += __popcll(bk);
        const unsigned long long bo = __ballot(out);
        if (bo) {
          int wpos = -1, wr = 0;
          q3_place(bo, lane, ltmask, d, pt, off, W.SB, cnt, mx, champ, cx, cy, cz, wpos, wr);
          if (wpos >= 0) W.sb[wpos] = wr;
        }
        hl_sync();
      }
      if (cnt) {
        if (off + cnt > W.SB) { S.status |= QHS_CAPACITY | Q3_CAPBIT(QHS_CAP_SB); return; }
        if (lane == 0) {
          W.sb[off + cnt - 1] = champ;
          W.soff[f] = off;
          W.fdist[f] = mx;
          q3_set_cc(W, L, f, (unsigned)cnt | ((unsigned)champ << 16));
        }
        S.sbtop += cnt;
      }
      np = w;
      hl_sync();
    }
    if (np > 0) {
      S.nnew = 4;
      if (lane == 0)
        for (int i = 0; i < 4; i++) {
          L.nslot[i] = fs[i];
          for (int k = 0; k < 4; k++) L.npl[4 * i + k] = q[i][k];
          L.nflag[i] = q3_fa(W, L, fs[i]);
          L.nn1[i] = L.nn2[i] = 0;
        }
      S.nmov = 0;
      S.findbestnew = 1;
      hl_sync();
      int rg;
      double rd;
      HullPt rpt, pre;
      pre.x = pre.y = pre.z = 0.0;
      pre.q = -1;
      pre.pad = 0;
      q3_locate_seq(W, S, L, np, 0, true, lane, pre, 0, false, rg, rd, rpt);
      q3_emit_seq(W, S, L, np, 0, true, lane, rg, rd, rpt);
      S.findbestnew = 0;
      S.nnew = 0;
      S.nmov = 0;
      hl_sync();
    }
    if (S.status & (QHS_INPUT | QHS_TOPOLOGY | QHS_CAPACITY)) return;
    {
      int order[4] = {fs[0], fs[1], fs[2], fs[3]};
      unsigned kk[4];
      for (int i = 0; i < 4; i++) kk[i] = q3_key(W, L, order[i]);
      for (int a = 0; a < 4; a++)
        for (int b = a + 1; b < 4; b++)
          if (kk[b] < kk[a]) {
            const unsigned tk = kk[a]; kk[a] = kk[b]; kk[b] = tk;
            const int to = order[a]; order[a] = order[b]; order[b] = to;
          }
      int best = -1;
      double bd = -DBL_MAX;
      for (int i = 0; i < 4; i++) {
        const int f = order[i];
        if ((q3_cc(W, L, f) & 0xffffu) && W.fdist[f] > bd) { best = f; bd = W.fdist[f]; }
      }
      hl_sync();
      if (best >= 0) {
        q3_set_key(W, L, best, 0u);
        for (int i = 0; i < 4; i++)
          if (order[i] == best) {
            for (int t = i; t > 0; t--) { order[t] = order[t - 1]; kk[t] = kk[t - 1]; }
            order[0] = best;
            kk[0] = 0;
            break;
          }
      }
      int qt = 0;
      for (int i = 0; i < 4; i++)
        if (q3_cc(W, L, order[i]) & 0xffffu) {
          if (lane == 0) {
            W.fq[qt] = order[i];
            W.fqk[qt] = kk[i];
            HullPt r;
            r.x = r.y = r.z = 0.0; r.q = -1; r.pad = 0;
            W.fqc[qt] = r;
          }
          qt++;
        }
      S.qhead = 0;
      S.qtail = qt;
      hl_sync();
    }
  }
  Q3T(0);
  if (lane == 0) {
    L.c_dist[0] = S.MINvisible; L.c_dist[1] = S.MAXcoplanar; L.c_dist[2] = S.DISTround;
    L.c_dist[3] = S.MINdenom; L.c_dist[4] = S.MINdenom_2;
    for (int k = 0; k < 3; k++) { L.c_dist[5 + k] = S.NEARzero[k]; L.c_interior[k] = S.interior[k]; }
  }
  int phase = 0;
  int qcb = 0, qcn = 0;
  int qf = 0, qp = -1;
  unsigned qk = 0;
  double qx = 0.0, qy = 0.0, qz = 0.0;
  for (;;) {
#ifdef LQRO_QHULL_PROFILE
    unsigned long long snap_[21];
    for (int k = 0; k < 21; k++) snap_[k] = S.tph[k];
#endif
    int facet = -1, furthest = -1;
    double apexp[3] = {0.0, 0.0, 0.0};
    bool adopt = false;
    bool pfv = false;
    bool fast = false;
    int nvis = 0, nnew = 0, lm = 0;
    const double* ncb = W.ncoord;
    HullPt pre;
    pre.x = pre.y = pre.z = 0.0;
    pre.q = -1;
    pre.pad = 0;
    int pfa = 0, pfnp = -1;
#ifdef LQRO_QHULL_LONGPROF
    const unsigned long long lp_ta = __builtin_amdgcn_s_memrealtime();
    S.lp_tail += S.lp_tw ? lp_ta - S.lp_tw : 0ull;
#endif
    if (phase > 0) {
#ifdef LQRO_QHULL_PROFILE
      const unsigned long long tw_ = __builtin_amdgcn_s_memtime();
#endif
#ifdef LQRO_QHULL_PROFILE
      int spins_ = 0;
      int dn = q3_ld_acq(&L.sp_done);
      const unsigned long long tf_ = __builtin_amdgcn_s_memtime();
      for (long w = 0; dn != phase && w < (1l << 24); ++w) {
        __builtin_amdgcn_s_sleep(Q3_W0_SLEEP);
        dn = q3_ld_acq(&L.sp_done);
        ++spins_;
      }
      if (S.prev1) { S.tfr += tf_ - tw_; S.nsp += (unsigned long long)spins_; }
#else
      const int dn = q3_wait(&L.sp_done, phase, false);
#endif
#ifdef LQRO_QHULL_LONGPROF
      {
        const unsigned long long tn = __builtin_amdgcn_s_memrealtime();
        const unsigned long long de = q3_lds(L.lp_doner);
        if (tn - lp_ta > 20 && tn > de && lane == 0) { L.hprof[6] += tn - de; L.hprof[7] += 1; }
      }
#endif
#ifdef LQRO_QHULL_PROFILE
      {
        const unsigned long long tn_ = __builtin_amdgcn_s_memtime();
        S.tw += tn_ - tw_;
        S.nw += 1;
        if (tn_ - tw_ > 200) S.tdl += tn_ - L.done_t;
        S.tseen = tn_;
        if (S.prev1) {
          S.tw1 += tn_ - tw_; S.nw1 += 1;
          S.tse += L.done_t - L.pub_t; S.tsn += tn_ - L.pub_t;
          S.tfr2 += L.done_t2 - L.pub_t;
          const unsigned long long nr_ = __builtin_amdgcn_s_memrealtime();
          S.r_start += L.start_r - L.pub_r; S.r_done += L.done_r - L.pub_r; S.r_seen += nr_ - L.pub_r;
        }
      }
#endif
#ifdef LQRO_QHULL_LONGPROF
      S.lp_wait += __builtin_amdgcn_s_memrealtime() - lp_ta;
#endif
      if (dn != phase) {
        S.status |= QHS_CAPACITY | QHS_TIMEOUT;
        return;
      }
      {
        const int sok = L.sp_ok, F = L.sp_facet, sfur = L.sp_furthest, spos = L.sp_pos;
        const int snv = L.sp_nvis, snn = L.sp_nnew, sst = L.sp_status;
        const unsigned skey = L.sp_key;
        const double sax = L.sp_apex[0], say = L.sp_apex[1], saz = L.sp_apex[2];
        const int vf = L.sp_visf[lane], vr = L.sp_repl[lane];
        const int vv0 = L.sp_vvert[3 * lane], vv1 = L.sp_vvert[3 * lane + 1], vv2 = L.sp_vvert[3 * lane + 2];
        const int t1 = L.sp_v1[lane], t2 = L.sp_v2[lane], thz = L.sp_nhz[lane], thk = L.sp_nhskip[lane];
        const int tfl = L.sp_nflag[lane], tn1 = L.sp_nn1[lane], tn2 = L.sp_nn2[lane];
        const double4 tpl = q3_lds(*reinterpret_cast<const double4*>(L.sp_npl + 4 * lane));
        const int oldv = lane < Q3_MOVCAP ? L.oldf[lane] : -1;
        const int pfd = hl_ld(&L.pf_done);
        hl_cfence();
        const int pso = L.pf_vsoff[lane], psc = L.pf_vscnt[lane], ppnp = L.pf_np, ppfa = L.pf_prea[lane];
        const HullPt ppre = L.pf_pre[lane];
        if (sok && F >= 0 && snv >= 1 && snv <= 64 && snn >= 1 && snn <= 64) {
          const unsigned c = q3_cc(W, L, F), k0 = q3_key(W, L, F);
          const int fa0 = q3_fa(W, L, F);
          int vfa = 0;
          unsigned vkey = 0u;
          if (lane < snv) { vfa = q3_fa(W, L, vf); vkey = q3_key(W, L, vf); }
          const int e = lane - snv;
          int fsl = 0;
          if (e >= 0 && e < S.nfs) fsl = L.fstk[S.nfs - 1 - e];
          adopt = (fa0 & QF_LIVE) && k0 == skey && (c & 0xffffu) > 0 && (int)(c >> 16) == sfur;
          if (adopt) {
            facet = F;
            furthest = sfur;
            apexp[0] = sax; apexp[1] = say; apexp[2] = saz;
            S.qhead = spos;
            q3_set_cc(W, L, F, (c & 0xffffu) - 1u);
            nvis = snv;
            nnew = snn;
            bool bad = false;
            if (lane < nvis) {
              bad = vkey >= S.key0_last;
              for (int t = 0; t < S.nold; t++) bad |= __builtin_amdgcn_readlane(oldv, t) == vf;
            }
            pfv = pfd == phase && __ballot(bad) == 0ull;
            if (lane < nvis) {
              int so = pso, sc = psc;
              if (!pfv) {
                so = W.soff[vf];
                sc = vf == F ? (int)((c & 0xffffu) - 1u) : (int)(q3_cc(W, L, vf) & 0xffffu);
              }
              L.visf[lane] = vf;
              L.repl[lane] = vr;
              q3_set_fa(W, L, vf, vfa | QF_VISIBLE);
              L.vvert[3 * lane] = vv0; L.vvert[3 * lane + 1] = vv1; L.vvert[3 * lane + 2] = vv2;
              L.vsoff[lane] = so;
              L.vscnt[lane] = sc;
            }
            if (lane < nnew) {
              L.nv[3 * lane] = furthest; L.nv[3 * lane + 1] = t1; L.nv[3 * lane + 2] = t2;
              L.nhz[lane] = thz;
              L.nhskip[lane] = thk;
              L.nflag[lane] = tfl;
              L.nn1[lane] = tn1;
              L.nn2[lane] = tn2;
              q3_lds_st(*reinterpret_cast<double4*>(L.npl + 4 * lane), tpl);
            }
            S.status |= sst;
            S.nvis = nvis;
            lm = sst & QHS_FLIPPED;
            ncb = W.ncoord2;
            fast = true;
            if (!(S.status & (QHS_TOPOLOGY | QHS_CAPACITY))) {
              S.nnew = nnew;
              if (pfv) { pfnp = ppnp; pre = ppre; pfa = ppfa; }
              const int extra = nnew > nvis ? nnew - nvis : 0;
              const int take = extra < S.nfs ? extra : S.nfs;
              if (S.nalloc + extra - take > W.FC) {
                S.status |= QHS_CAPACITY | Q3_CAPBIT(QHS_CAP_FACETS);
              } else {
                const int slot = lane < nvis ? vf : (e < S.nfs ? fsl : S.nalloc + (e - S.nfs));
                if (lane < nnew) L.nslot[lane] = slot;
                S.nfs -= take;
                S.nalloc += extra - take;
                const unsigned key0 = S.keyc;
                const int s1 = __builtin_amdgcn_ds_bpermute(tn1 << 2, slot);
                const int s2 = __builtin_amdgcn_ds_bpermute(tn2 << 2, slot);
                if (lane < nnew) {
                  const double q[4] = {tpl.x, tpl.y, tpl.z, tpl.w};
                  q3_set_facet(W, L, slot, q, thz, s1, s2, tfl | (lane << 8));
                  q3_set_key(W, L, slot, key0 + (unsigned)lane);
                  q3_set_cc(W, L, slot, 0u);
                  q3_set_nb(W, L, thz, thk, slot);
                }
                S.keyc += (unsigned)nnew;
                S.key0_last = key0;
              }
            }
            hl_sync();
          }
        }
      }
      if (!fast && L.sp_ok) {
        const int F = L.sp_facet;
        const unsigned c = q3_cc(W, L, F);
        adopt = (q3_fa(W, L, F) & QF_LIVE) && q3_key(W, L, F) == L.sp_key && (c & 0xffffu) > 0 &&
                (int)(c >> 16) == L.sp_furthest;
        if (adopt) {
          facet = F;
          furthest = L.sp_furthest;
          apexp[0] = L.sp_apex[0]; apexp[1] = L.sp_apex[1]; apexp[2] = L.sp_apex[2];
          S.qhead = L.sp_pos;
          hl_sync();
          q3_set_cc(W, L, facet, (c & 0xffffu) - 1u);
          hl_sync();
        }
      }
    }
    while (!adopt && S.qhead < S.qtail) {
      if (S.qhead >= qcb + qcn) {
        qcb = S.qhead;
        qcn = min(64, S.qtail - S.qhead);
        if (lane < qcn) {
          qf = W.fq[qcb + lane];
          qk = W.fqk[qcb + lane];
          const HullPt e = W.fqc[qcb + lane];
          qx = e.x; qy = e.y; qz = e.z; qp = e.q;
        }
      }
      bool ok = false;
      unsigned c = 0;
      if (lane < qcn && qcb + lane >= S.qhead) {
        const int fa = q3_fa(W, L, qf);
        c = q3_cc(W, L, qf);
        ok = (fa & QF_LIVE) && q3_key(W, L, qf) == qk && (c & 0xffffu) > 0;
      }
      const unsigned long long b = __ballot(ok);
      if (b) {
        const int l = __ffsll((long long)b) - 1;
        S.qhead = qcb + l;
        facet = __builtin_amdgcn_readlane(qf, l);
        const unsigned cf = (unsigned)__builtin_amdgcn_readlane((int)c, l);
        furthest = (int)(cf >> 16);
        if (__builtin_amdgcn_readlane(qp, l) == furthest) {
          apexp[0] = hl_rl(qx, l); apexp[1] = hl_rl(qy, l); apexp[2] = hl_rl(qz, l);
        } else {
          apexp[0] = W.Pr[3 * (size_t)furthest];
          apexp[1] = W.Pr[3 * (size_t)furthest + 1];
          apexp[2] = W.Pr[3 * (size_t)furthest + 2];
        }
        hl_sync();
        q3_set_cc(W, L, facet, (cf & 0xffffu) - 1u);
        hl_sync();
        break;
      }
      S.qhead = qcb + qcn;
    }
    Q3T(1);
#ifdef LQRO_QHULL_PROFILE
    const unsigned long long tins_ = S.tq;
#endif
    if (furthest < 0) {
      if (phase > 0 && q3_wait(&L.sp_gdone, phase, false) != phase) S.status |= QHS_CAPACITY | QHS_TIMEOUT;
      break;
    }
    int ts = 0, my_t = -1;
    bool one = false;
    double P1[3] = {0.0, 0.0, 0.0}, P2[3] = {0.0, 0.0, 0.0}, PO[3] = {0.0, 0.0, 0.0};
    if (fast) {
    } else if (adopt) {
      nvis = L.sp_nvis;
      nnew = L.sp_nnew;
      const bool pfr = q3_ld_acq(&L.pf_done) == phase;
      if (nvis <= 64) {
        int f = 0, rp = 0, v0 = 0, v1 = 0, v2 = 0, pso = 0, psc = 0, fa = 0;
        unsigned key = 0u;
        bool bad = false;
        if (lane < nvis) {
          f = L.sp_visf[lane];
          rp = L.sp_repl[lane];
          v0 = L.sp_vvert[3 * lane]; v1 = L.sp_vvert[3 * lane + 1]; v2 = L.sp_vvert[3 * lane + 2];
          pso = L.pf_vsoff[lane];
          psc = L.pf_vscnt[lane];
          fa = q3_fa(W, L, f);
          key = q3_key(W, L, f);
          bad = key >= S.key0_last;
          for (int t = 0; t < S.nold; t++) bad |= L.oldf[t] == f;
        }
        pfv = pfr && __ballot(bad) == 0ull;
        if (lane < nvis) {
          int so = pso, sc = psc;
          if (!pfv) {
            so = W.soff[f];
            sc = (int)(q3_cc(W, L, f) & 0xffffu);
          }
          L.visf[lane] = f;
          L.repl[lane] = rp;
          q3_set_fa(W, L, f, fa | QF_VISIBLE);
          L.vvert[3 * lane] = v0; L.vvert[3 * lane + 1] = v1; L.vvert[3 * lane + 2] = v2;
          L.vsoff[lane] = so;
          L.vscnt[lane] = sc;
        }
      } else {
        for (int vi = lane; vi < nvis; vi += 64) {
          const int f = L.sp_visf[vi];
          L.visf[vi] = f;
          L.repl[vi] = L.sp_repl[vi];
          q3_set_fa(W, L, f, q3_fa(W, L, f) | QF_VISIBLE);
          L.vvert[3 * vi] = L.sp_vvert[3 * vi]; L.vvert[3 * vi + 1] = L.sp_vvert[3 * vi + 1];
          L.vvert[3 * vi + 2] = L.sp_vvert[3 * vi + 2];
          L.vsoff[vi] = W.soff[f];
          L.vscnt[vi] = (int)(q3_cc(W, L, f) & 0xffffu);
        }
      }
      for (int t = lane; t < nnew; t += 64) {
        const int a1 = L.sp_v1[t], a2 = L.sp_v2[t], hz = L.sp_nhz[t], hk = L.sp_nhskip[t], fl = L.sp_nflag[t];
        const int m1 = L.sp_nn1[t], m2 = L.sp_nn2[t];
        const double4 pl = q3_lds(*reinterpret_cast<const double4*>(L.sp_npl + 4 * t));
        L.nv[3 * t] = furthest; L.nv[3 * t + 1] = a1; L.nv[3 * t + 2] = a2;
        L.nhz[t] = hz;
        L.nhskip[t] = hk;
        L.nflag[t] = fl;
        L.nn1[t] = m1;
        L.nn2[t] = m2;
        q3_lds_st(*reinterpret_cast<double4*>(L.npl + 4 * t), pl);
      }
      S.status |= L.sp_status;
      S.nvis = nvis;
      lm = L.sp_status & QHS_FLIPPED;
      ncb = W.ncoord2;
      hl_sync();
      Q3T(2);
    } else {
    if (phase > 0 && q3_wait(&L.sp_gdone, phase, false) != phase) {
      S.status |= QHS_CAPACITY | QHS_TIMEOUT;
      return;
    }
    {
      const int fa0 = q3_fa(W, L, facet);
      hl_sync();
      if (lane == 0) L.visf[0] = facet;
      q3_set_fa(W, L, facet, fa0 | QF_VISIBLE);
      hl_sync();
    }
    int ls = 0;
    nvis = 1;
    for (int lo = 0; lo < nvis;) {
      const int hi = nvis;
      const int ncand = 3 * (hi - lo);
      for (int c0 = 0; c0 < ncand; c0 += 64) {
        const int c = c0 + lane;
        int nb = -1, fa = QF_VISIBLE;
        double q[4] = {0.0, 0.0, 0.0, 0.0};
        if (c < ncand) {
          nb = q3_nb(W, L, L.visf[lo + c / 3], c % 3);
          int nn[3];
          q3_get(W, L, nb, q, nn, &fa);
        }
        const bool cand = !(fa & QF_VISIBLE);
        const double dist = cand ? q3_distq(q, apexp) : 0.0;
        bool vis = cand && dist >= S.MINvisible;
        if (cand && !vis && dist >= -S.MAXcoplanar) ls |= QHS_COPLANAR;
        bool dup = false;
        for (unsigned long long mm = __ballot(vis); mm;) {
          const int l = __ffsll((long long)mm) - 1;
          mm &= mm - 1;
          dup |= (l < lane) && __builtin_amdgcn_readlane(nb, l) == nb;
        }
        vis = vis && !dup;
        const unsigned long long bv = __ballot(vis);
        if (vis) {
          const int at = nvis + __popcll(bv & ltmask);
          if (at < Q3_VISCAP) L.visf[at] = nb;
          q3_set_fa(W, L, nb, fa | QF_VISIBLE);
        }
        nvis += __popcll(bv);
        hl_sync();
      }
      lo = hi;
      if (nvis > Q3_VISCAP) { S.status |= QHS_CAPACITY | Q3_CAPBIT(QHS_CAP_VIS); return; }
    }
    S.status |= qh_wave_or(ls);
    S.nvis = nvis;
    Q3T(2);
    for (int vi = lane; vi < nvis; vi += 64) L.repl[vi] = -1;
    hl_sync();
    one = 3 * nvis <= 64;
    for (int c0 = 0; c0 < 3 * nvis; c0 += 64) {
      const int c = c0 + lane;
      int vis = -1, nb = -1, hfa = QF_VISIBLE;
      int hn[3] = {-1, -1, -1};
      if (c < 3 * nvis) {
        const int vi = c / 3;
        vis = L.visf[vi];
        nb = q3_nb(W, L, vis, c - 3 * vi);
        q3_tp(W, L, nb, hn, &hfa);
        if (c == 3 * vi) {
          const Q3V& vw = W.vv[vis];
          L.vvert[3 * vi] = vw.id[0]; L.vvert[3 * vi + 1] = vw.id[1]; L.vvert[3 * vi + 2] = vw.id[2];
          L.vsoff[vi] = W.soff[vis];
          L.vscnt[vi] = (int)(q3_cc(W, L, vis) & 0xffffu);
        }
      }
      const bool ridge = !(hfa & QF_VISIBLE);
      const unsigned long long b = __ballot(ridge);
      if (ridge) {
        const int t = nnew + __popcll(b & ltmask);
        const int hskip = hn[0] == vis ? 0 : hn[1] == vis ? 1 : hn[2] == vis ? 2 : -1;
        if (hskip < 0) {
          ts |= QHS_TOPOLOGY;
        } else if (t < Q3_NEWCAP) {
          const Q3V& h = W.vv[nb];
          const int top = (hfa & QF_TOP) ? (hskip & 1) : ((hskip & 1) ^ 1);
          const int i1 = hskip == 0 ? 1 : 0, i2 = hskip == 2 ? 1 : 2;
          double p1[3], p2[3], po[3];
          for (int k = 0; k < 3; k++) {
            p1[k] = h.p[3 * i1 + k];
            p2[k] = h.p[3 * i2 + k];
            po[k] = h.p[3 * hskip + k];
          }
          L.nv[3 * t] = furthest;
          L.nv[3 * t + 1] = h.id[i1];
          L.nv[3 * t + 2] = h.id[i2];
          L.nhz[t] = nb;
          L.nhskip[t] = hskip;
          atomicMax(&L.repl[c / 3], t);
          double q[4];
          bool flipped;
          int fl = QF_NEW | QF_LIVE | (top ? QF_TOP : 0);
          q3_plane(S, lm, apexp, p1, p2, top, q, &flipped);
          if (flipped) { fl |= QF_FLIPPED; lm |= QHS_FLIPPED; }
          L.nflag[t] = fl;
          L.npl[4 * t] = q[0]; L.npl[4 * t + 1] = q[1]; L.npl[4 * t + 2] = q[2]; L.npl[4 * t + 3] = q[3];
          if (one) {
            my_t = t;
            for (int k = 0; k < 3; k++) { P1[k] = p1[k]; P2[k] = p2[k]; PO[k] = po[k]; }
          } else {
            for (int k = 0; k < 3; k++) {
              W.ncoord[9 * t + k] = p1[k]; W.ncoord[9 * t + 3 + k] = p2[k]; W.ncoord[9 * t + 6 + k] = po[k];
            }
          }
        }
      }
      nnew += __popcll(b);
    }
    Q3T(19);
    }
    S.status |= qh_wave_or(ts);
    if (nnew > Q3_NEWCAP) S.status |= QHS_CAPACITY | Q3_CAPBIT(QHS_CAP_NEW);
    if (S.status & (QHS_TOPOLOGY | QHS_CAPACITY)) return;
    S.nnew = nnew;
    hl_sync();
    if (pfv && !fast) {
      pfnp = L.pf_np;
      pre = L.pf_pre[lane];
      pfa = L.pf_prea[lane];
    }
    if (!fast) {
      const int extra = nnew > nvis ? nnew - nvis : 0;
      const int take = extra < S.nfs ? extra : S.nfs;
      if (S.nalloc + extra - take > W.FC) { S.status |= QHS_CAPACITY | Q3_CAPBIT(QHS_CAP_FACETS); return; }
      for (int t = lane; t < nnew; t += 64) L.nslot[t] = q3_alloc(S, L, t);
      S.nfs -= take;
      S.nalloc += extra - take;
      hl_sync();
    }
    Q3T(3);
    const unsigned key0 = S.keyc;
    auto finish = [&](int t, const double* p1, const double* p2) {
      int nbu[2] = {-1, -1};
      if (adopt) {
        nbu[0] = L.nn1[t];
        nbu[1] = L.nn2[t];
      } else {
        int cnt[2] = {0, 0};
        const int w0 = L.nv[3 * t + 2], w1 = L.nv[3 * t + 1];
#pragma unroll 4
        for (int u = 0; u < nnew; u++) {
          const int a = L.nv[3 * u + 1], b = L.nv[3 * u + 2];
          const bool o = u != t;
          if (o && (a == w0 || b == w0)) { nbu[0] = u; cnt[0]++; }
          if (o && (a == w1 || b == w1)) { nbu[1] = u; cnt[1]++; }
        }
        if (cnt[0] != 1 || cnt[1] != 1) lm |= QHS_TOPOLOGY;
        L.nn1[t] = nbu[0] >= 0 ? nbu[0] : 0;
        L.nn2[t] = nbu[1] >= 0 ? nbu[1] : 0;
      }
      const int s = L.nslot[t];
      const double4 q4 = q3_lds(*reinterpret_cast<const double4*>(L.npl + 4 * t));
      const int hz = L.nhz[t], hk = L.nhskip[t], fl = L.nflag[t], id1 = L.nv[3 * t + 1], id2 = L.nv[3 * t + 2];
      const int s1 = nbu[0] >= 0 ? L.nslot[nbu[0]] : 0, s2 = nbu[1] >= 0 ? L.nslot[nbu[1]] : 0;
      const double q[4] = {q4.x, q4.y, q4.z, q4.w};
      q3_set_facet(W, L, s, q, hz, s1, s2, fl | (t << 8));
      q3_set_key(W, L, s, key0 + (unsigned)t);
      q3_set_cc(W, L, s, 0u);
      if (!adopt) {
        Q3V& v = W.vv[s];
        *reinterpret_cast<double4*>(v.p) = make_double4(apexp[0], apexp[1], apexp[2], p1[0]);
        *reinterpret_cast<double4*>(v.p + 4) = make_double4(p1[1], p1[2], p2[0], p2[1]);
        *reinterpret_cast<double2*>(v.p + 8) = make_double2(p2[2], 0.0);
        *reinterpret_cast<int4*>(v.id) = make_int4(furthest, id1, id2, 0);
      }
      q3_set_nb(W, L, hz, hk, s);
    };
    if (fast) {
    } else if (one) {
      if (my_t >= 0) finish(my_t, P1, P2);
    } else {
      for (int t = lane; t < nnew; t += 64) {
        double p1[3] = {0.0, 0.0, 0.0}, p2[3] = {0.0, 0.0, 0.0};
        if (!adopt)
          for (int k = 0; k < 3; k++) { p1[k] = ncb[9 * t + k]; p2[k] = ncb[9 * t + 3 + k]; }
        finish(t, p1, p2);
      }
    }
    if (!fast) {
      S.keyc += (unsigned)nnew;
      S.key0_last = key0;
    }
    hl_sync();
    if (!adopt && !(qh_wave_or(lm) & QHS_FLIPPED)) {
      auto zero = [&](int t, const double* p1, const double* p2, const double* po) {
        const double d1 = q3_distq(L.npl + 4 * L.nn1[t], p1);
        const double d2 = q3_distq(L.npl + 4 * L.nn2[t], p2);
        const double d3 = q3_distq(L.npl + 4 * t, po);
        if (d1 >= -2 * S.DISTround || d2 >= -2 * S.DISTround || d3 >= -2 * S.DISTround) lm |= QHS_NONCONVEX;
      };
      if (one) {
        if (my_t >= 0) zero(my_t, P1, P2, PO);
      } else {
        for (int t = lane; t < nnew; t += 64) {
          double p1[3], p2[3], po[3];
          for (int k = 0; k < 3; k++) {
            p1[k] = ncb[9 * t + k]; p2[k] = ncb[9 * t + 3 + k]; po[k] = ncb[9 * t + 6 + k];
          }
          zero(t, p1, p2, po);
        }
      }
    }
    S.status |= qh_wave_or(lm);
    Q3T(4);
    if (S.status & (QHS_TOPOLOGY | QHS_CAPACITY)) return;
    hl_sync();
    if (lane == 0) {
      L.pub_qhead = S.qhead;
      L.pub_qtail = S.qtail;
      L.pub_adopt = adopt ? 1 : 0;
      L.pub_nnew = nnew;
    }
    ++phase;
#ifdef LQRO_QHULL_PROFILE
    if (lane == 0) { L.pub_t = __builtin_amdgcn_s_memtime(); L.pub_r = __builtin_amdgcn_s_memrealtime(); }
    if (S.tseen) { S.tpre += __builtin_amdgcn_s_memtime() - S.tseen; S.npre += 1; }
#endif
#ifdef LQRO_QHULL_LONGPROF
    const unsigned long long lp_t0 = __builtin_amdgcn_s_memrealtime();
    S.lp_adopt += lp_t0 - lp_ta;
    if (lane == 0) L.lp_pubr = lp_t0;
#endif
    if (lane == 0) q3_st_rel(&L.ph, phase);
#ifdef LQRO_QHULL_PROFILE
    if (lane == 0) S.trel += __builtin_amdgcn_s_memtime() - L.pub_t;
#endif
    S.findbestnew = 0;
    S.notsharp = 0;
    S.nmov = 0;
    int np2 = 0;
    for (int c0 = 0; c0 < nvis; c0 += 64) {
      const int vi = c0 + lane;
      const int cnt = vi < nvis ? L.vscnt[vi] : 0;
      const int inc = q3_scan_add(cnt);
      if (vi < nvis) L.vinc[vi] = np2 + inc;
      np2 += __builtin_amdgcn_readlane(inc, 63);
    }
    hl_sync();
    int prestart = 0;
    if (pfv && np2 == pfnp) {
      if (lane < np2) prestart = L.repl[pfa] >= 0 ? L.repl[pfa] : 0;
    } else if (lane < np2) {
      pre = q3_seqpt(W, L, nvis, false, lane, &prestart);
    }
    Q3T(5);
    const int sharp = adopt ? L.sp_sharp : q3_sharpnewfacets(S, L, lane);
    Q3T(20);
    Q3C(21, 1);
    S.nins++;
    Q3C(31, adopt ? 1 : 0);
    Q3C(22, np2);
    if (np2) {
      int rg;
      double rd;
      HullPt rpt;
      q3_locate_seq(W, S, L, np2, sharp, false, lane, pre, prestart, true, rg, rd, rpt);
#ifdef LQRO_QHULL_LONGPROF
      if (np2 > 64) S.lp_tloc += __builtin_amdgcn_s_memrealtime() - lp_t0;
#endif
      Q3T(6);
      q3_emit_seq(W, S, L, np2, nnew, false, lane, rg, rd, rpt);
      Q3T(7);
    }
#ifdef LQRO_QHULL_LONGPROF
    {
      const unsigned long long dt = __builtin_amdgcn_s_memrealtime() - lp_t0;
      S.lp_all += dt;
      if (np2 > 64) { S.lp_n += 1; S.lp_pts += (unsigned long long)np2; S.lp_t += dt; }
      S.lp_tw = lp_t0 + dt;
    }
#endif
    if (S.status & QHS_CAPACITY) return;
    if (nnew != nvis + 2) {
      int lsd = 0;
      for (int t = lane; t < 3 * nvis; t += 64) {
        const int v = L.vvert[t];
        bool skip = false;
        for (int u = 0; u < nnew && !skip; u++) skip = L.nv[3 * u + 1] == v || L.nv[3 * u + 2] == v;
        for (int e = 0; e < t && !skip; e++) skip = L.vvert[e] == v;
        if (skip) continue;
        const double p[3] = {W.Pr[3 * (size_t)v], W.Pr[3 * (size_t)v + 1], W.Pr[3 * (size_t)v + 2]};
        double d;
        int iso, trig;
        q3_locate<false>(W, S, L, p, 0, 2, &d, &iso, &trig, lsd, q3_col0(L, lane));
        if (d >= -S.MAXcoplanar) lsd |= QHS_COPLANAR;
      }
      S.status |= qh_wave_or(lsd);
    }
    Q3T(8);
    if (S.status & QHS_CAPACITY) return;
    for (int t = nnew + lane; t < nvis; t += 64) {
      const int f = L.visf[t];
      q3_set_fa(W, L, f, 0);
      const int at = S.nfs + (t - nnew);
      if (at < Q3_FSTK) L.fstk[at] = (unsigned short)f;
    }
    if (nvis > nnew) S.nfs = min(Q3_FSTK, S.nfs + (nvis - nnew));
    for (int t = lane; t < nnew; t += 64) q3_set_fa(W, L, L.nslot[t], L.nflag[t] & ~QF_NEW);
    S.nnew = 0;
    S.nmov = 0;
    S.findbestnew = 0;
    S.notsharp = 0;
    hl_sync();
    Q3T(9);
#ifdef LQRO_QHULL_PROFILE
    S.prev1 = np2 <= 64;
    if (np2 > 64) { S.tph[29] += S.tq - tins_; S.tph[30] += 1; }
    else {
      for (int k = 0; k < 21; k++) S.tps[k] += S.tph[k] - snap_[k];
      S.nps += 1;
    }
#endif
  }
}

__device__ inline bool q3_merge_suspect(const Q3W& W, const Q3L& L, const Q3S& S, int lane, const double* vrel,
                                        double best, int head) {
  const double T = -LQRO_QHMERGE_K * S.DISTround;
  bool sus = false;
  for (int f0 = 1; f0 < S.nalloc; f0 += 64) {
    const int f = f0 + lane;
    double q[4] = {0.0, 0.0, 0.0, 0.0};
    bool con = false;
    if (f < S.nalloc && (q3_fa(W, L, f) & QF_LIVE)) {
      q3_pl(W, L, f, q);
      const double* P = W.Pf + 3 * (size_t)W.vv[f].id[0];
      con = fabs(q[0] * (vrel[0] - P[0]) + q[1] * (vrel[1] - P[1]) + q[2] * (vrel[2] - P[2])) <= best + 1e-6 ||
            f == head;
    }
    unsigned long long m = __ballot(con);
    while (m) {
      const int src = __ffsll((long long)m) - 1;
      m &= m - 1;
      const int fc = __shfl(f, src);
      double qc[4];
      for (int k = 0; k < 4; k++) qc[k] = __shfl(q[k], src);
      const int a = W.vv[fc].id[0], b = W.vv[fc].id[1], c = W.vv[fc].id[2];
      for (int g = 1 + lane; g < S.nalloc; g += 64) {
        if (!(q3_fa(W, L, g) & QF_LIVE)) continue;
        for (int t = 0; t < 3; t++) {
          const int id = W.vv[g].id[t];
          if (id == a || id == b || id == c) continue;
          if (q3_distq(qc, W.Pr + 3 * (size_t)id) >= T) sus = true;
        }
      }
    }
  }
  return __ballot(sus) != 0;
}

__device__ inline bool q3_select(const HullArgs& A, const Q3W& W, const Q3L& L, const Q3S& S, int lane,
                                 const double* xi, const double* vrel, int slot) {
  const bool fail = (S.status & (QHS_INPUT | QHS_TOPOLOGY | QHS_CAPACITY)) != 0;
  double ub = INFINITY;
  unsigned minkey = 0xffffffffu;
  int nfac = 0, head = -1;
  if (!fail) {
    for (int f0 = 1; f0 < S.nalloc; f0 += 256) {
      int fs[4], fa[4], v[4];
#pragma unroll
      for (int u = 0; u < 4; u++) {
        fs[u] = f0 + 64 * u + lane;
        fa[u] = fs[u] < S.nalloc ? q3_fa(W, L, fs[u]) : 0;
        v[u] = (fa[u] & QF_LIVE) ? W.vv[fs[u]].id[0] : 0;
      }
#pragma unroll
      for (int u = 0; u < 4; u++) {
        if (!(fa[u] & QF_LIVE)) continue;
        const int f = fs[u];
        nfac++;
        const unsigned k = q3_key(W, L, f);
        if (k < minkey) { minkey = k; head = f; }
        double q[4];
        q3_pl(W, L, f, q);
        const double* P = W.Pf + 3 * (size_t)v[u];
        double b;
        const double d = qsel_dist(q, P, vrel, &b);
        ub = fmin(ub, d + b);
      }
    }
  }
  for (int off = 32; off >= 1; off >>= 1) {
    const unsigned om = (unsigned)__shfl_xor((int)minkey, off);
    const int oh = __shfl_xor(head, off);
    nfac += __shfl_xor(nfac, off);
    if (om < minkey) { minkey = om; head = oh; }
    ub = fmin(ub, __shfl_xor(ub, off));
  }
  double best = INFINITY, bn[3] = {0.0, 0.0, 0.0};
  unsigned bkey = 0xffffffffu;
  int bf = -1;
  if (!fail) {
    for (int f = 1 + lane; f < S.nalloc; f += 64) {
      if (!(q3_fa(W, L, f) & QF_LIVE)) continue;
      double q[4];
      q3_pl(W, L, f, q);
      const double* P = W.Pf + 3 * (size_t)W.vv[f].id[0];
      double b;
      const double d0 = qsel_dist(q, P, vrel, &b);
      if (d0 - b > ub) continue;
      double n16[3];
      const double d = qsel_dist16(q, P, vrel, n16);
      const unsigned k = q3_key(W, L, f);
      if (d < best || (d == best && k < bkey)) {
        best = d; bkey = k; bf = f;
        bn[0] = n16[0]; bn[1] = n16[1]; bn[2] = n16[2];
      }
    }
  }
  for (int off = 32; off >= 1; off >>= 1) {
    const double ob = __shfl_xor(best, off);
    const unsigned ok = (unsigned)__shfl_xor((int)bkey, off);
    const int of = __shfl_xor(bf, off);
    const double o0 = __shfl_xor(bn[0], off), o1 = __shfl_xor(bn[1], off), o2 = __shfl_xor(bn[2], off);
    if (ob < best || (ob == best && ok < bkey)) { best = ob; bkey = ok; bf = of; bn[0] = o0; bn[1] = o1; bn[2] = o2; }
  }
  const bool ok = !fail && nfac > 0 && bf >= 0;
  const bool stale = ok && bkey == minkey;
  const bool merged = (S.status & (QHS_COPLANAR | QHS_NONCONVEX | QHS_FLIPPED | QHS_NARROW | QHS_SINGULAR)) != 0;
  const bool mwin = ok && merged && q3_merge_suspect(W, L, S, lane, vrel, best, head);
  int bv[3] = {0, 0, 0};
  if (ok)
    for (int t = 0; t < 3; t++) bv[t] = W.vv[bf].id[t];
  int go = 0;
  if (lane == 0) {
    float* pl = A.planes + (size_t)slot * 8;
    double* qn = A.qnrm + (size_t)slot * 4;
    double nrm[3] = {0.0, 0.0, 0.0};
    if (ok && !stale) {
      nrm[0] = bn[0]; nrm[1] = bn[1]; nrm[2] = bn[2];
      const double dh = best * 0.5;
      const double mult = 1.0;
      pl[0] = (float)(xi[3] + mult * dh * nrm[0]);
      pl[1] = (float)(xi[4] + mult * dh * nrm[1]);
      pl[2] = (float)(xi[5] + mult * dh * nrm[2]);
      pl[3] = (float)nrm[0]; pl[4] = (float)nrm[1]; pl[5] = (float)nrm[2];
      pl[6] = __int_as_float(1);
      qn[0] = nrm[0]; qn[1] = nrm[1]; qn[2] = nrm[2]; qn[3] = best;
      atomicAdd(&A.stats[3], 1ull);
    } else if (stale) {
      pl[6] = __int_as_float(3);
      qn[0] = qn[1] = qn[2] = 0.0; qn[3] = best;
      const int k = atomicAdd(A.qstale_count, 1);
      if (k < A.qstale_cap) A.qstale[k] = slot;
      atomicAdd(&A.stats[3], 1ull);
    } else {
      pl[6] = __int_as_float(0);
      hull_fail_note(A.stats, slot);
    }
    if (ok && merged) atomicAdd(&A.stats[LQRO_ST_MERGED], 1ull);
    if (mwin) qhmerge_note(A.stats, slot);
    if (A.recs) {
      lqro_pair_record& rec = A.recs[slot];
      rec.flags |= ok ? LQRO_REC_HULL : LQRO_REC_HULLFAIL;
      if (stale) rec.flags |= LQRO_REC_STALE;
      if (merged) rec.flags |= LQRO_REC_QHMERGE;
      if (mwin) rec.flags |= LQRO_REC_QHMERGE_WIN;
      rec.n_facets = ok ? nfac : -(S.status & 0xffff) - 1;
      if (ok) {
        rec.facet[0] = bv[0]; rec.facet[1] = bv[1]; rec.facet[2] = bv[2];
        rec.dist = best;
        for (int q = 0; q < 3; ++q) {
          rec.normal[q] = nrm[q];
          rec.plane_point[q] = stale ? 0.0f : pl[q];
          rec.plane_normal[q] = stale ? 0.0f : pl[3 + q];
        }
      }
    }
    go = hull_row_done(A, slot, stale, A.row_lp != 0);
  }
  hl_sync();
  return __builtin_amdgcn_readfirstlane(go) != 0;
}

__device__ inline void q3_row_lp(const HullArgs& A, Q3L& L, int slot, int lane) {
  static_assert(sizeof(L.pl) >= 2 * LQRO_EARLY_LP_MAX_NPR * 32, "q3_row_lp: the planes must fit");
  const int lrow = slot / A.npr;
  const int i = A.row_begin + lrow * A.row_stride;
  float* planes = reinterpret_cast<float*>(L.pl);
  float* proj = planes + (size_t)A.npr * 8;
  __threadfence();
  const int m = lp_compact<8>(A.planes + (size_t)lrow * A.npr * 8, A.npr, planes, lane);
  const v3 pref = V3((float)A.lp_vgoal[3 * i], (float)A.lp_vgoal[3 * i + 1], (float)A.lp_vgoal[3 * i + 2]);
  v3 nv = V3(0.0f, 0.0f, 0.0f);
  const int fail = w_lp3<8>(planes, m, A.lp_vmax, pref, false, nv, lane);
  if (fail < m) w_lp4<8>(planes, m, fail, (float)A.lp_vmax, nv, proj, lane);
  if (lane == 0) {
    A.lp_newv[3 * i] = nv.x;
    A.lp_newv[3 * i + 1] = nv.y;
    A.lp_newv[3 * i + 2] = nv.z;
  }
  hl_sync();
}

#ifdef LQRO_QBIG_NOINLINE
__device__ __attribute__((noinline)) void q3_big_inline(const HullArgs& A, QhL& LB, int slot, unsigned long long tjob,
                                                        int wave) {
#else
__device__ inline void q3_big_inline(const HullArgs& A, QhL& LB, int slot, unsigned long long tjob, int wave) {
#endif
  const int lane = threadIdx.x & 63;
  const int HNP = A.H * A.NP;
  const QhW W = qh_worker(A.qscratch + (size_t)(A.block_base + blockIdx.x) * A.qstride, HNP);
  const int lrow = slot / A.npr, jj = A.nbr_list ? A.nbr_list[slot] : slot % A.npr;
  const int i = A.row_begin + lrow * A.row_stride;
  const int j = jj < i ? jj : jj + 1;
  const double* xi = A.x + (size_t)i * A.X;
  const double* xj = A.x + (size_t)j * A.X;
  const double* Ti = A.T + (A.per_agent ? (size_t)i * A.H * 9 : 0);
  const double* Ni = A.NCF + (A.per_agent ? (size_t)i * A.H * 3 * A.X : 0);
  const double vrel[3] = {xi[3] - xj[3], xi[4] - xj[4], xi[5] - xj[5]};
  const int n = hull_points(A, LB, Ti, Ni, xi, xj, vrel, W.Pr, W.Pf);
  unsigned* owner = qw_owner(A.qscratch + (size_t)(A.block_base + blockIdx.x) * A.qstride, A.qstride);
  if (wave == 0) {
    qh_claim_scratch(W, owner, lane);
    QhS S;
#ifdef LQRO_QHULL_PROFILE
    for (int k = 0; k < 12; k++) S.tph[k] = 0;
#endif
    S.status = 0;
    S.nalloc = 1;
    S.nins = 0;
    S.facet_list = S.facet_tail = 0;
    if (LB.fail || n < 4) S.status = QHS_INPUT;
    else qh_build(W, S, LB, n, lane);
    hl_sync();
    qh_select(A, W, S, lane, xi, vrel, slot);
    if (lane == 0) hull_build_note(A, slot, 1, tjob, n, S.nins, S.nalloc - 1);
  }
}

__device__ __forceinline__ void q3_body(const HullArgs& A, Q3L& L, QhL* LB = nullptr) {
  const int lane = threadIdx.x & 63;
  const int wave = __builtin_amdgcn_readfirstlane(threadIdx.x >> 6);
  const int HNP = A.H * A.NP;
  const Q3W W = q3_worker(A.qscratch + (size_t)(A.block_base + blockIdx.x) * A.qstride, HNP);
  for (;;) {
    const int slot = hull_take_job(A, L, false);
    if (slot < 0) break;
    const unsigned long long tjob = __builtin_amdgcn_s_memrealtime();
    const bool spec = A.spec_mark != nullptr && A.spec_mark[slot] >= 2;
    if (threadIdx.x == 0) {
      L.ph = 0; L.sp_done = 0; L.sp_gdone = 0; L.hctl = 0u; L.hbusy = 0; L.sp_hz = 0; L.pf_done = 0;
      L.ectl = 0u; L.edone = 0;
      L.qflags = A.qflags;
#ifdef LQRO_QHULL_LONGPROF
      for (int k = 0; k < 12; k++) L.hprof[k] = 0ull;
      L.lp_pubr = L.lp_doner = 0ull;
#endif
      L.big_slot = -1;
    }
    for (int q = threadIdx.x; q < Q3_FL / 2; q += blockDim.x) reinterpret_cast<unsigned*>(L.mark)[q] = 0u;
    const int lrow = slot / A.npr, jj = A.nbr_list ? A.nbr_list[slot] : slot % A.npr;
    const int i = A.row_begin + lrow * A.row_stride;
    const int j = jj < i ? jj : jj + 1;
    const double* xi = A.x + (size_t)i * A.X;
    const double* xj = A.x + (size_t)j * A.X;
    const double* Ti = A.T + (A.per_agent ? (size_t)i * A.H * 9 : 0);
    const double* Ni = A.NCF + (A.per_agent ? (size_t)i * A.H * 3 * A.X : 0);
    const double vrel[3] = {xi[3] - xj[3], xi[4] - xj[4], xi[5] - xj[5]};
    const int n = hull_points(A, L, Ti, Ni, xi, xj, vrel, W.Pr, W.Pf);
    bool lp_go = false;
    if (wave >= 2) {
      const Q3Col CH = q3_colh(W, wave, lane);
      int last = 0;
      long idle = 0;
      for (;;) {
        if (wave == 2) {
          const int hz = q3_ld_acq(&L.sp_hz);
          if (hz != last && hz > 0) {
            last = hz;
            q3_prefetch(W, L, lane, hz);
            idle = 0;
            continue;
          }
        }
        if (q3_help(W, L, lane, CH)) { idle = 0; continue; }
        if (q3_emit_help(W, L, lane)) { idle = 0; continue; }
        if (q3_ld_acq(&L.ph) < 0) break;
        if (++idle > (1l << 24)) break;
        __builtin_amdgcn_s_sleep(Q3_W2_SLEEP);
      }
    } else if (wave == 1) {
      unsigned* owner = qw_owner(A.qscratch + (size_t)(A.block_base + blockIdx.x) * A.qstride, A.qstride);
      if (*owner != QW_OWNER_Q3) {
        for (int q = lane; q < W.FC; q += 64) W.mark2[q] = 0u;
        if (lane == 0) { W.ctr[0] = 0u; *owner = QW_OWNER_Q3; }
      }
      unsigned ep2 = W.ctr[0];
      unsigned short ep = 0;
      const Q3Col CH = q3_colh(W, 1, lane);
      int last = 0;
      Q3QC Q;
      Q.qcb = 0; Q.qcn = 0; Q.qf = 0; Q.qp = -1; Q.qk = 0u; Q.qx = Q.qy = Q.qz = 0.0;
      Q.pc_from = -1; Q.pc_pos = -1; Q.pc_end = 0; Q.pc_f = 0; Q.pc_p = -1; Q.pc_k = 0u;
      Q.pc_x = Q.pc_y = Q.pc_z = 0.0;
      Q.one = 0; Q.rt = -1;
      for (int k = 0; k < 6; k++) Q.r[k] = 0.0;
      long idle = 0;
      Q3P P;
      for (int k = 0; k < 16; k++) P.t[k] = 0;
      for (;;) {
        const int p = q3_ld_acq(&L.ph);
        if (p != last) {
          if (p < 0) break;
          last = p;
          ++ep;
          ++ep2;
#ifdef LQRO_QHULL_PROFILE
          const unsigned long long t0_ = __builtin_amdgcn_s_memtime();
          P.tq = t0_;
          P.t[14] += t0_ - L.pub_t;
          if (P.tq2) P.t[15] += t0_ - P.tq2;
          if (lane == 0) L.start_r = __builtin_amdgcn_s_memrealtime();
#endif
#ifdef LQRO_QHULL_LONGPROF
          const unsigned long long ts_ = __builtin_amdgcn_s_memrealtime();
#endif
          q3_spec(W, L, lane, ep, ep2, Q, P, p);
          hl_sync();
#ifdef LQRO_QHULL_LONGPROF
          if (lane == 0) {
            const unsigned long long te_ = __builtin_amdgcn_s_memrealtime();
            L.hprof[3] += 1; L.hprof[4] += ts_ - q3_lds(L.lp_pubr); L.hprof[5] += te_ - ts_;
            L.lp_doner = te_;
          }
#endif
#ifdef LQRO_QHULL_PROFILE
          if (lane == 0) L.done_t = __builtin_amdgcn_s_memtime();
#endif
          if (lane == 0) q3_st_rel_lds(&L.sp_done, p);
          if (lane == 0) q3_st_rel(&L.sp_gdone, p);
          if (L.qflags & 4) q3_prescan(W, L, lane, ep, ep2, Q);
#ifdef LQRO_QHULL_PROFILE
          if (lane == 0) { L.done_t2 = __builtin_amdgcn_s_memtime(); L.done_r = __builtin_amdgcn_s_memrealtime(); }
          P.tq2 = __builtin_amdgcn_s_memtime();
          P.t[0] += __builtin_amdgcn_s_memtime() - t0_;
          P.t[7] += 1;
#endif
          idle = 0;
          continue;
        }
        {
#ifdef LQRO_QHULL_PROFILE
          const unsigned long long t0_ = __builtin_amdgcn_s_memtime();
#endif
          if (q3_help(W, L, lane, CH)) {
#ifdef LQRO_QHULL_PROFILE
            P.t[6] += __builtin_amdgcn_s_memtime() - t0_;
            P.t[8] += 1;
#endif
            idle = 0;
            continue;
          }
        }
        if (q3_emit_help(W, L, lane)) { idle = 0; continue; }
        if (++idle > (1l << 24)) break;
        __builtin_amdgcn_s_sleep(Q3_W1_SLEEP);
      }
#ifdef LQRO_QHULL_PROFILE
      if (A.prof && lane == 0)
        for (int k = 0; k < 16; k++) atomicAdd(&A.prof[Q3_PROF_W1 + k], P.t[k]);
#endif
      if (lane == 0) W.ctr[0] = ep2;
    } else {
    Q3S S;
#ifdef LQRO_QHULL_PROFILE
    for (int k = 0; k < 32; k++) S.tph[k] = 0;
    S.tw = S.nw = 0;
    S.tdl = 0;
    S.tw1 = S.nw1 = 0;
    S.tse = S.tsn = 0;
    S.tfr = S.nsp = 0;
    S.tfr2 = 0;
    S.trel = 0;
    S.r_start = S.r_done = S.r_seen = S.r_gseen = 0;
    S.tseen = S.tpre = S.npre = S.tstart = 0;
    S.prev1 = 0;
    for (int k = 0; k < 24; k++) S.tps[k] = 0;
    S.nps = 0;
    const unsigned long long tjob_ = __builtin_amdgcn_s_memtime();
#endif
    S.status = 0;
    S.nalloc = 1;
    S.nins = 0;
    S.lp_n = S.lp_pts = S.lp_t = S.lp_all = S.lp_tloc = S.lp_wait = S.lp_adopt = S.lp_tail = S.lp_tw = 0;
    S.lp_own = S.lp_got = S.lp_hwait = S.lp_stop = S.lp_ev = S.lp_posts = 0;
    if (L.fail || n < 4) S.status = QHS_INPUT;
    else q3_build(W, S, L, n, lane);
    hl_sync();
    if (lane == 0) q3_st_rel(&L.ph, -1);
    bool keep = true;
    if (spec) {
      int m = 0;
      if (lane == 0) {
        m = __hip_atomic_load(A.spec_mark + slot, __ATOMIC_ACQUIRE, __HIP_MEMORY_SCOPE_AGENT);
        for (long w = 0; m == 2 && w < (1l << 26); ++w) {
          __builtin_amdgcn_s_sleep(8);
          m = __hip_atomic_load(A.spec_mark + slot, __ATOMIC_ACQUIRE, __HIP_MEMORY_SCOPE_AGENT);
        }
        if (m == 2) {
          atomicAdd(&A.stats[LQRO_ST_TIMEOUT], 1ull);
          hull_fail_note(A.stats, slot);
        }
      }
      keep = __builtin_amdgcn_readfirstlane(m) == 3;
    }
    if (!keep) {
    } else if (S.status & QHS_CAPACITY) {
      if (lane == 0) {
        atomicAdd(&A.stats[LQRO_ST_RETRY], 1ull);
        if (S.status & QHS_TIMEOUT) atomicAdd(&A.stats[LQRO_ST_TIMEOUT], 1ull);
        if (LB) {
          L.big_slot = slot;
        } else {
          const int r = atomicAdd(A.rcount, 1);
          if (r < A.cap) A.rqueue[r] = slot;
        }
        hull_build_note(A, slot, 2, tjob, n, S.nins, S.nalloc - 1);
#ifdef LQRO_QHULL_PROFILE
        if (A.prof) {
          const unsigned long long k = atomicAdd(&A.prof[Q3_PROF_RETRY], 1ull);
          atomicOr(&A.prof[Q3_PROF_RETRY + 1], (unsigned long long)S.status);
          if (k < 14) A.prof[Q3_PROF_RETRY + 2 + k] = (unsigned long long)slot | ((unsigned long long)S.status << 32);
        }
#endif
      }
      hl_sync();
    } else {
#ifdef LQRO_QHULL_PROFILE
    unsigned long long tq_ = __builtin_amdgcn_s_memtime();
#endif
    lp_go = q3_select(A, W, L, S, lane, xi, vrel, slot);
    if (lane == 0) {
      const int k = hull_build_note(A, slot, 0, tjob, n, S.nins, S.nalloc - 1);
#ifdef LQRO_QHULL_LONGPROF
      if (A.prof && k >= 0 && k < 1024) {
        unsigned long long* r = A.prof + Q3_PROF_LONG + 24 * k;
        r[0] = S.lp_n; r[1] = S.lp_pts; r[2] = S.lp_t; r[3] = S.lp_all;
        r[4] = S.lp_tloc; r[5] = S.lp_wait; r[6] = S.lp_adopt - S.lp_wait; r[7] = S.lp_tail;
        r[8] = S.lp_own; r[9] = S.lp_got; r[10] = S.lp_hwait; r[11] = S.lp_stop; r[12] = S.lp_ev; r[13] = S.lp_posts;
        r[14] = L.hprof[0]; r[15] = L.hprof[1] | (L.hprof[2] << 32);
        for (int q = 3; q < 11; q++) r[13 + q] = L.hprof[q];
      }
#else
      (void)k;
#endif
    }
#ifdef LQRO_QHULL_PROFILE
    S.tph[10] = __builtin_amdgcn_s_memtime() - tq_;
    S.tph[27] = __builtin_amdgcn_s_memtime() - tjob_;
    S.tph[28] = (unsigned long long)n;
    if (A.prof && lane == 0) {
      for (int k = 0; k < 32; k++)
        if (k != 26 && k != 11) atomicAdd(&A.prof[k], S.tph[k]);
      atomicAdd(&A.prof[Q3_PROF_W1 + 9], S.tw);
      atomicAdd(&A.prof[Q3_PROF_W1 + 10], S.nw);
      for (int k = 0; k < 24; k++) atomicAdd(&A.prof[Q3_PROF_W1 + 16 + k], S.tps[k]);
      atomicAdd(&A.prof[Q3_PROF_W1 + 40], S.nps);
      atomicAdd(&A.prof[Q3_PROF_W1 + 41], S.tdl);
      atomicAdd(&A.prof[Q3_PROF_W1 + 42], S.tw1);
      atomicAdd(&A.prof[Q3_PROF_W1 + 43], S.nw1);
      atomicAdd(&A.prof[Q3_PROF_W1 + 44], S.tse);
      atomicAdd(&A.prof[Q3_PROF_W1 + 45], S.tsn);
      atomicAdd(&A.prof[Q3_PROF_W1 + 46], S.tfr);
      atomicAdd(&A.prof[Q3_PROF_W1 + 47], S.nsp);
      atomicAdd(&A.prof[Q3_PROF_W1 + 48], S.tfr2);
      atomicAdd(&A.prof[Q3_PROF_W1 + 49], S.trel);
      atomicAdd(&A.prof[Q3_PROF_W1 + 50], S.r_start);
      atomicAdd(&A.prof[Q3_PROF_W1 + 51], S.r_done);
      atomicAdd(&A.prof[Q3_PROF_W1 + 52], S.r_seen);
      atomicAdd(&A.prof[Q3_PROF_W1 + 53], S.r_gseen);
      atomicAdd(&A.prof[Q3_PROF_W1 + 54], S.tpre);
      atomicAdd(&A.prof[Q3_PROF_W1 + 55], S.npre);
      atomicAdd(&A.prof[Q3_PROF_W1 + 56], S.tstart);
      atomicMax(&A.prof[26], S.tph[27]);
      const unsigned long long j = atomicAdd(&A.prof[11], 1ull);
      if (j < 4096) {
        A.prof[32 + 2 * j] = S.tph[27];
        A.prof[33 + 2 * j] = S.tph[21] | ((unsigned long long)n << 20) | ((unsigned long long)S.nalloc << 40);
      }
    }
#endif
    if (A.ext_nf && lane == 0) *A.ext_nf = S.status;
    if (A.ext_facets) {
      for (int f = 1 + lane; f < S.nalloc; f += 64) {
        if (!(q3_fa(W, L, f) & QF_LIVE)) continue;
        const unsigned k = q3_key(W, L, f);
        int rank = 0, nl = 0;
        for (int g = 1; g < S.nalloc; g++)
          if (q3_fa(W, L, g) & QF_LIVE) { nl++; rank += q3_key(W, L, g) < k; }
        if (rank < A.ext_max)
          for (int t = 0; t < 3; t++) A.ext_facets[3 * rank + t] = W.vv[f].id[t];
        if (rank == 0 && nl < A.ext_max) A.ext_facets[3 * nl] = -1;
      }
      hl_sync();
    }
    }
    }
#ifndef LQRO_QHULL_NO_INLINE_BIG
    if (LB) {
      __syncthreads();
      const int bs = L.big_slot;
      __syncthreads();
      if (bs >= 0) {
        q3_big_inline(A, *LB, bs, tjob, wave);
        __syncthreads();
      }
    }
#endif
    if (A.rowpend) {
      __syncthreads();
      if (wave == 0 && lp_go) q3_row_lp(A, L, slot, lane);
    }
  }
}

}
```

Measured before the change: 59.53 million.

## Replace per-facet global vertex-coordinate records with packed 16-bit vertex ids

Removes the global Q3V array, which cached each facet's three vertex coordinates and ids, and instead stores the three vertex ids packed as 16-bit values in LDS, or in the spill record's former padding. Coordinates are re-read from the point array when needed. Several LDS index arrays shrink to 16-bit, and Q3_FL is lowered to fit the new arrays. The cross-wave sp_gdone wait and the helper-side vv write-back on adoption are dropped, cutting global stores and a synchronization point. The cost is extra indirect global loads of point coordinates during horizon processing, fewer facets kept in LDS, and an implicit limit of 65536 vertex ids.

```diff
diff --git a/lqr-obstacles_amd/csrc/lqro_qhull3.hpp b/lqr-obstacles_amd/csrc/lqro_qhull3.hpp
--- a/lqr-obstacles_amd/csrc/lqro_qhull3.hpp
+++ b/lqr-obstacles_amd/csrc/lqro_qhull3.hpp
@@ -27,7 +27,7 @@
 #define Q3_W2_SLEEP 1
 #endif
 #ifndef Q3_FL
-#define Q3_FL 2240
+#define Q3_FL 2120
 #endif
 #define Q3_PROF_RETRY (32 + 2 * 4096 + 16)
 #ifdef LQRO_QHULL_PROFILE
@@ -42,20 +42,14 @@
   int fa;
   unsigned key;
   unsigned cc;
-  int pad[2];
+  unsigned vid01, vid2;
 };
-
-struct Q3V {
-  double p[9];
-  double pad;
-  int id[4];
-};
+static_assert(sizeof(Q3G) == 64, "a spilled facet slot is one 64-byte record");
 
 struct Q3W {
   double* Pr;
   double* Pf;
   Q3G* G;
-  Q3V* vv;
   double* ncoord;
   int* soff;
   double* fdist;
@@ -79,7 +73,7 @@
 __host__ __device__ inline size_t q3_worker_bytes(int HNP) {
   const size_t FC = 2 * (size_t)HNP + Q3_NEWCAP + 16, SB = (size_t)QH_SBMULT * HNP, QC = 4 * (size_t)HNP + 64;
   const size_t NG = FC > Q3_FL ? FC - Q3_FL : 1;
-  return q3_align(24 * (size_t)HNP) * 2 + q3_align(64 * NG) + q3_align(96 * FC) + q3_align(72 * Q3_NEWCAP) +
+  return q3_align(24 * (size_t)HNP) * 2 + q3_align(64 * NG) + q3_align(72 * Q3_NEWCAP) +
          q3_align(4 * FC) +
          q3_align(8 * FC) + q3_align(4 * SB) + q3_align(4 * (size_t)HNP) * 2 + q3_align(8 * (size_t)HNP) +
          q3_align(4 * QC) * 2 + q3_align(32 * QC) + q3_align(72 * Q3_NEWCAP) + q3_align(4 * FC) + 256 +
@@ -98,7 +92,6 @@
   W.Pr = reinterpret_cast<double*>(take(24 * (size_t)HNP));
   W.Pf = reinterpret_cast<double*>(take(24 * (size_t)HNP));
   W.G = reinterpret_cast<Q3G*>(take(64 * NG));
-  W.vv = reinterpret_cast<Q3V*>(take(96 * (size_t)W.FC));
   W.ncoord = reinterpret_cast<double*>(take(72 * (size_t)Q3_NEWCAP));
   W.soff = reinterpret_cast<int*>(take(4 * (size_t)W.FC));
   W.fdist = reinterpret_cast<double*>(take(8 * (size_t)W.FC));
@@ -128,15 +121,17 @@
   ushort4 tp[Q3_FL];
   unsigned key[Q3_FL];
   unsigned cc[Q3_FL];
+  unsigned vid01[Q3_FL];
+  unsigned short vid2[Q3_FL];
   unsigned short fstk[Q3_FSTK];
-  int visf[Q3_VISCAP];
+  unsigned short visf[Q3_VISCAP];
   int vsoff[Q3_VISCAP], vscnt[Q3_VISCAP], vinc[Q3_VISCAP];
-  int vvert[3 * Q3_VISCAP];
+  unsigned short vvert[3 * Q3_VISCAP];
   int repl[Q3_VISCAP];
-  int nslot[Q3_NEWCAP];
-  int nv[3 * Q3_NEWCAP];
-  int nhz[Q3_NEWCAP], nhskip[Q3_NEWCAP];
-  int nn1[Q3_NEWCAP], nn2[Q3_NEWCAP];
+  unsigned short nslot[Q3_NEWCAP];
+  unsigned short nv[3 * Q3_NEWCAP];
+  unsigned short nhz[Q3_NEWCAP], nhskip[Q3_NEWCAP];
+  unsigned short nn1[Q3_NEWCAP], nn2[Q3_NEWCAP];
   alignas(32) double npl[4 * Q3_NEWCAP];
   int nflag[Q3_NEWCAP];
   int movf[Q3_MOVCAP];
@@ -146,11 +141,12 @@
   double dchp[3 * Q3_ND];
   int cop[Q3_COPCAP * 64];
   unsigned short hvis[Q3_HZCAP * 64];
-  int sp_visf[Q3_VISCAP];
+  unsigned short sp_visf[Q3_VISCAP];
   int sp_repl[Q3_VISCAP];
-  int sp_v1[Q3_NEWCAP], sp_v2[Q3_NEWCAP], sp_nhz[Q3_NEWCAP], sp_nhskip[Q3_NEWCAP], sp_nflag[Q3_NEWCAP];
-  int sp_nn1[Q3_NEWCAP], sp_nn2[Q3_NEWCAP];
-  int sp_vvert[3 * Q3_VISCAP];
+  unsigned short sp_v1[Q3_NEWCAP], sp_v2[Q3_NEWCAP], sp_nhz[Q3_NEWCAP], sp_nhskip[Q3_NEWCAP];
+  int sp_nflag[Q3_NEWCAP];
+  unsigned short sp_nn1[Q3_NEWCAP], sp_nn2[Q3_NEWCAP];
+  unsigned short sp_vvert[3 * Q3_VISCAP];
   alignas(32) double sp_npl[4 * Q3_NEWCAP];
   unsigned short mark[Q3_FL];
   unsigned short sp_cand[3 * Q3_VISCAP];
@@ -162,10 +158,9 @@
   double c_dist[8];
   double c_interior[3];
   int ph, sp_done, sp_ok, sp_facet, sp_furthest, sp_pos, sp_nvis, sp_nnew, sp_status, sp_sharp;
-  int sp_gdone;
   unsigned sp_key;
   int pub_qhead, pub_qtail;
-  int pub_adopt, pub_nnew;
+  int pub_adopt;
   double hr_d[Q3_HR * 64];
   unsigned short hr_f[Q3_HR * 64];
   unsigned short hr_k[Q3_HR * 64];
@@ -381,6 +376,48 @@
     q3_glb_st(*reinterpret_cast<double4*>(g.pl), make_double4(q[0], q[1], q[2], q[3]));
     q3_glb_st(*reinterpret_cast<int4*>(g.nb), make_int4(nb0, nb1, nb2, fa));
   }
+}
+__device__ __forceinline__ void q3_vid(const Q3W& W, const Q3L& L, int f, int* id) {
+  if (f < Q3_FL) {
+    const unsigned a = q3_lds(L.vid01[f]);
+    id[2] = q3_lds(L.vid2[f]);
+    id[0] = (int)(a & 0xffffu); id[1] = (int)(a >> 16);
+  } else {
+    const q3_v2u a = *(const Q3_AS1 q3_v2u*)(&W.G[f - Q3_FL].vid01);
+    id[0] = (int)(a.x & 0xffffu); id[1] = (int)(a.x >> 16); id[2] = (int)(a.y & 0xffffu);
+  }
+}
+__device__ __forceinline__ int q3_vid0(const Q3W& W, const Q3L& L, int f) {
+  return (int)((f < Q3_FL ? q3_lds(L.vid01[f]) : q3_glb(W.G[f - Q3_FL].vid01)) & 0xffffu);
+}
+__device__ __forceinline__ void q3_set_vid(const Q3W& W, Q3L& L, int f, int id0, int id1, int id2) {
+  const unsigned a = (unsigned)id0 | ((unsigned)id1 << 16);
+  if (f < Q3_FL) {
+    q3_lds_st(L.vid01[f], a);
+    q3_lds_st(L.vid2[f], (unsigned short)id2);
+  } else {
+    q3_v2u t; t.x = a; t.y = (unsigned)id2;
+    *(Q3_AS1 q3_v2u*)(&W.G[f - Q3_FL].vid01) = t;
+  }
+}
+__device__ __forceinline__ void q3_tpv(const Q3W& W, const Q3L& L, int f, int* nb, int* fa, int* id) {
+  if (f < Q3_FL) {
+    const ushort4 t = q3_lds(L.tp[f]);
+    const unsigned a = q3_lds(L.vid01[f]);
+    id[2] = q3_lds(L.vid2[f]);
+    nb[0] = t.x; nb[1] = t.y; nb[2] = t.z; *fa = t.w;
+    id[0] = (int)(a & 0xffffu); id[1] = (int)(a >> 16);
+  } else {
+    const Q3G& g = W.G[f - Q3_FL];
+    const int4 t = q3_glb(*reinterpret_cast<const int4*>(g.nb));
+    const q3_v2u a = *(const Q3_AS1 q3_v2u*)(&g.vid01);
+    nb[0] = t.x; nb[1] = t.y; nb[2] = t.z; *fa = t.w;
+    id[0] = (int)(a.x & 0xffffu); id[1] = (int)(a.x >> 16); id[2] = (int)(a.y & 0xffffu);
+  }
+}
+__device__ __forceinline__ void q3_pr(const Q3W& W, int id, double* p) {
+  const double* r = W.Pr + 3 * (size_t)id;
+  p[0] = q3_glb(r[0]); p[1] = q3_glb(r[1]); p[2] = q3_glb(r[2]);
 }
 
 __device__ __forceinline__ QhS q3_as_qhs(const Q3S& S) {
@@ -1340,8 +1377,6 @@
   int qcb, qcn, qf, qp;
   unsigned qk;
   double qx, qy, qz;
-  int one, rt;
-  double r[6];
   int pc_from, pc_pos, pc_end, pc_f, pc_p;
   unsigned pc_k;
   double pc_x, pc_y, pc_z;
@@ -1361,30 +1396,6 @@
     if (f < Q3_FL) q3_lds_st(L.mark[f], ep);
     else q3_glb_st(W.mark2[f], ep2);
   };
-  if (L.pub_adopt) {
-    const int nn = L.pub_nnew;
-    if (Q.one) {
-      if (Q.rt >= 0) {
-        const int t = Q.rt;
-        Q3V& v = W.vv[L.nslot[t]];
-        *reinterpret_cast<double4*>(v.p) = make_double4(L.sp_apex[0], L.sp_apex[1], L.sp_apex[2], Q.r[0]);
-        *reinterpret_cast<double4*>(v.p + 4) = make_double4(Q.r[1], Q.r[2], Q.r[3], Q.r[4]);
-        *reinterpret_cast<double2*>(v.p + 8) = make_double2(Q.r[5], 0.0);
-        *reinterpret_cast<int4*>(v.id) = make_int4(L.nv[3 * t], L.nv[3 * t + 1], L.nv[3 * t + 2], 0);
-      }
-    } else {
-      for (int t = lane; t < nn; t += 64) {
-        Q3V& v = W.vv[L.nslot[t]];
-        const double* nc = W.ncoord2 + 9 * t;
-        *reinterpret_cast<double4*>(v.p) = make_double4(L.sp_apex[0], L.sp_apex[1], L.sp_apex[2], nc[0]);
-        *reinterpret_cast<double4*>(v.p + 4) = make_double4(nc[1], nc[2], nc[3], nc[4]);
-        *reinterpret_cast<double2*>(v.p + 8) = make_double2(nc[5], 0.0);
-        *reinterpret_cast<int4*>(v.id) = make_int4(L.nv[3 * t], L.nv[3 * t + 1], L.nv[3 * t + 2], 0);
-      }
-    }
-  }
-  Q.one = 0;
-  Q.rt = -1;
   W1T(1);
 #ifdef LQRO_QHULL_LONGPROF
   const unsigned long long tq0_ = __builtin_amdgcn_s_memrealtime();
@@ -1537,16 +1548,18 @@
         const int c = c0 + lane;
         int vis = -1, nb = -1, hfa = 0;
         bool ridge = false;
-        int hn[3] = {-1, -1, -1};
+        int hn[3] = {-1, -1, -1}, hid[3] = {0, 0, 0};
         if (c < 3 * nvis) {
           const int vi = c / 3;
           vis = L.sp_visf[vi];
           nb = L.sp_cand[c];
-          q3_tp(W, L, nb, hn, &hfa);
+          q3_tpv(W, L, nb, hn, &hfa, hid);
           ridge = !marked(nb);
           if (c == 3 * vi) {
-            const Q3V& vw = W.vv[vis];
-            L.sp_vvert[3 * vi] = vw.id[0]; L.sp_vvert[3 * vi + 1] = vw.id[1]; L.sp_vvert[3 * vi + 2] = vw.id[2];
+            int vw[3];
+            q3_vid(W, L, vis, vw);
+            L.sp_vvert[3 * vi] = (unsigned short)vw[0]; L.sp_vvert[3 * vi + 1] = (unsigned short)vw[1];
+            L.sp_vvert[3 * vi + 2] = (unsigned short)vw[2];
           }
         }
         const unsigned long long b = __ballot(ridge);
@@ -1557,19 +1570,17 @@
           if (hskip < 0) {
             ts |= QHS_TOPOLOGY;
           } else if (t < Q3_NEWCAP) {
-            const Q3V& h = W.vv[nb];
             const int top = (hfa & QF_TOP) ? (hskip & 1) : ((hskip & 1) ^ 1);
-            const int i1 = hskip == 0 ? 1 : 0, i2 = hskip == 2 ? 1 : 2;
+            const int id1 = hskip == 0 ? hid[1] : hid[0], id2 = hskip == 2 ? hid[1] : hid[2];
+            const int ido = hskip == 0 ? hid[0] : hskip == 1 ? hid[1] : hid[2];
             double p1[3], p2[3], po[3];
-            for (int k = 0; k < 3; k++) {
-              p1[k] = h.p[3 * i1 + k];
-              p2[k] = h.p[3 * i2 + k];
-              po[k] = h.p[3 * hskip + k];
-            }
-            L.sp_v1[t] = h.id[i1];
-            L.sp_v2[t] = h.id[i2];
-            L.sp_nhz[t] = nb;
-            L.sp_nhskip[t] = hskip;
+            q3_pr(W, id1, p1);
+            q3_pr(W, id2, p2);
+            q3_pr(W, ido, po);
+            L.sp_v1[t] = (unsigned short)id1;
+            L.sp_v2[t] = (unsigned short)id2;
+            L.sp_nhz[t] = (unsigned short)nb;
+            L.sp_nhskip[t] = (unsigned short)hskip;
             atomicMax(&L.sp_repl[c / 3], t);
             double q[4];
             bool flipped;
@@ -1580,8 +1591,8 @@
             L.sp_npl[4 * t] = q[0]; L.sp_npl[4 * t + 1] = q[1]; L.sp_npl[4 * t + 2] = q[2]; L.sp_npl[4 * t + 3] = q[3];
             if (one) {
               my_t = t;
-              rv1 = h.id[i1];
-              rv2 = h.id[i2];
+              rv1 = id1;
+              rv2 = id2;
               for (int k = 0; k < 4; k++) Q4[k] = q[k];
               for (int k = 0; k < 3; k++) { P1[k] = p1[k]; P2[k] = p2[k]; PO[k] = po[k]; }
             } else {
@@ -1594,11 +1605,6 @@
         nnew += __popcll(b);
       }
       ok = nnew <= Q3_NEWCAP;
-      if (one) {
-        Q.one = 1;
-        Q.rt = my_t;
-        for (int k = 0; k < 3; k++) { Q.r[k] = P1[k]; Q.r[3 + k] = P2[k]; }
-      }
       W1T(4);
       if (ok) {
         hl_sync();
@@ -1937,11 +1943,7 @@
                      QF_LIVE | (tops[i] ? QF_TOP : 0) | (fl[i] ? QF_FLIPPED : 0));
         q3_set_key(W, L, f, S.keyc + i);
         q3_set_cc(W, L, f, 0u);
-        Q3V& v = W.vv[f];
-        for (int t = 0; t < 3; t++) {
-          for (int k = 0; k < 3; k++) v.p[3 * t + k] = W.Pr[3 * (size_t)fv[i][t] + k];
-          v.id[t] = fv[i][t];
-        }
+        q3_set_vid(W, L, f, fv[i][0], fv[i][1], fv[i][2]);
       }
     S.keyc += 4;
     hl_sync();
@@ -2093,7 +2095,6 @@
     bool pfv = false;
     bool fast = false;
     int nvis = 0, nnew = 0, lm = 0;
-    const double* ncb = W.ncoord;
     HullPt pre;
     pre.x = pre.y = pre.z = 0.0;
     pre.q = -1;
@@ -2214,7 +2215,6 @@
             S.status |= sst;
             S.nvis = nvis;
             lm = sst & QHS_FLIPPED;
-            ncb = W.ncoord2;
             fast = true;
             if (!(S.status & (QHS_TOPOLOGY | QHS_CAPACITY))) {
               S.nnew = nnew;
@@ -2236,6 +2236,7 @@
                   q3_set_facet(W, L, slot, q, thz, s1, s2, tfl | (lane << 8));
                   q3_set_key(W, L, slot, key0 + (unsigned)lane);
                   q3_set_cc(W, L, slot, 0u);
+                  q3_set_vid(W, L, slot, furthest, t1, t2);
                   q3_set_nb(W, L, thz, thk, slot);
                 }
                 S.keyc += (unsigned)nnew;
@@ -2305,10 +2306,7 @@
 #ifdef LQRO_QHULL_PROFILE
     const unsigned long long tins_ = S.tq;
 #endif
-    if (furthest < 0) {
-      if (phase > 0 && q3_wait(&L.sp_gdone, phase, false) != phase) S.status |= QHS_CAPACITY | QHS_TIMEOUT;
-      break;
-    }
+    if (furthest < 0) break;
     int ts = 0, my_t = -1;
     bool one = false;
     double P1[3] = {0.0, 0.0, 0.0}, P2[3] = {0.0, 0.0, 0.0}, PO[3] = {0.0, 0.0, 0.0};
@@ -2373,14 +2371,9 @@
       S.status |= L.sp_status;
       S.nvis = nvis;
       lm = L.sp_status & QHS_FLIPPED;
-      ncb = W.ncoord2;
       hl_sync();
       Q3T(2);
     } else {
-    if (phase > 0 && q3_wait(&L.sp_gdone, phase, false) != phase) {
-      S.status |= QHS_CAPACITY | QHS_TIMEOUT;
-      return;
-    }
     {
       const int fa0 = q3_fa(W, L, facet);
       hl_sync();
@@ -2434,15 +2427,17 @@
     for (int c0 = 0; c0 < 3 * nvis; c0 += 64) {
       const int c = c0 + lane;
       int vis = -1, nb = -1, hfa = QF_VISIBLE;
-      int hn[3] = {-1, -1, -1};
+      int hn[3] = {-1, -1, -1}, hid[3] = {0, 0, 0};
       if (c < 3 * nvis) {
         const int vi = c / 3;
         vis = L.visf[vi];
         nb = q3_nb(W, L, vis, c - 3 * vi);
-        q3_tp(W, L, nb, hn, &hfa);
+        q3_tpv(W, L, nb, hn, &hfa, hid);
         if (c == 3 * vi) {
-          const Q3V& vw = W.vv[vis];
-          L.vvert[3 * vi] = vw.id[0]; L.vvert[3 * vi + 1] = vw.id[1]; L.vvert[3 * vi + 2] = vw.id[2];
+          int vw[3];
+          q3_vid(W, L, vis, vw);
+          L.vvert[3 * vi] = (unsigned short)vw[0]; L.vvert[3 * vi + 1] = (unsigned short)vw[1];
+          L.vvert[3 * vi + 2] = (unsigned short)vw[2];
           L.vsoff[vi] = W.soff[vis];
           L.vscnt[vi] = (int)(q3_cc(W, L, vis) & 0xffffu);
         }
@@ -2455,20 +2450,18 @@
         if (hskip < 0) {
           ts |= QHS_TOPOLOGY;
         } else if (t < Q3_NEWCAP) {
-          const Q3V& h = W.vv[nb];
           const int top = (hfa & QF_TOP) ? (hskip & 1) : ((hskip & 1) ^ 1);
-          const int i1 = hskip == 0 ? 1 : 0, i2 = hskip == 2 ? 1 : 2;
+          const int id1 = hskip == 0 ? hid[1] : hid[0], id2 = hskip == 2 ? hid[1] : hid[2];
+          const int ido = hskip == 0 ? hid[0] : hskip == 1 ? hid[1] : hid[2];
           double p1[3], p2[3], po[3];
-          for (int k = 0; k < 3; k++) {
-            p1[k] = h.p[3 * i1 + k];
-            p2[k] = h.p[3 * i2 + k];
-            po[k] = h.p[3 * hskip + k];
-          }
-          L.nv[3 * t] = furthest;
-          L.nv[3 * t + 1] = h.id[i1];
-          L.nv[3 * t + 2] = h.id[i2];
-          L.nhz[t] = nb;
-          L.nhskip[t] = hskip;
+          q3_pr(W, id1, p1);
+          q3_pr(W, id2, p2);
+          q3_pr(W, ido, po);
+          L.nv[3 * t] = (unsigned short)furthest;
+          L.nv[3 * t + 1] = (unsigned short)id1;
+          L.nv[3 * t + 2] = (unsigned short)id2;
+          L.nhz[t] = (unsigned short)nb;
+          L.nhskip[t] = (unsigned short)hskip;
           atomicMax(&L.repl[c / 3], t);
           double q[4];
           bool flipped;
@@ -2512,7 +2505,7 @@
     }
     Q3T(3);
     const unsigned key0 = S.keyc;
-    auto finish = [&](int t, const double* p1, const double* p2) {
+    auto finish = [&](int t) {
       int nbu[2] = {-1, -1};
       if (adopt) {
         nbu[0] = L.nn1[t];
@@ -2539,25 +2532,14 @@
       q3_set_facet(W, L, s, q, hz, s1, s2, fl | (t << 8));
       q3_set_key(W, L, s, key0 + (unsigned)t);
       q3_set_cc(W, L, s, 0u);
-      if (!adopt) {
-        Q3V& v = W.vv[s];
-        *reinterpret_cast<double4*>(v.p) = make_double4(apexp[0], apexp[1], apexp[2], p1[0]);
-        *reinterpret_cast<double4*>(v.p + 4) = make_double4(p1[1], p1[2], p2[0], p2[1]);
-        *reinterpret_cast<double2*>(v.p + 8) = make_double2(p2[2], 0.0);
-        *reinterpret_cast<int4*>(v.id) = make_int4(furthest, id1, id2, 0);
-      }
+      q3_set_vid(W, L, s, furthest, id1, id2);
       q3_set_nb(W, L, hz, hk, s);
     };
     if (fast) {
     } else if (one) {
-      if (my_t >= 0) finish(my_t, P1, P2);
+      if (my_t >= 0) finish(my_t);
     } else {
-      for (int t = lane; t < nnew; t += 64) {
-        double p1[3] = {0.0, 0.0, 0.0}, p2[3] = {0.0, 0.0, 0.0};
-        if (!adopt)
-          for (int k = 0; k < 3; k++) { p1[k] = ncb[9 * t + k]; p2[k] = ncb[9 * t + 3 + k]; }
-        finish(t, p1, p2);
-      }
+      for (int t = lane; t < nnew; t += 64) finish(t);
     }
     if (!fast) {
       S.keyc += (unsigned)nnew;
@@ -2577,7 +2559,7 @@
         for (int t = lane; t < nnew; t += 64) {
           double p1[3], p2[3], po[3];
           for (int k = 0; k < 3; k++) {
-            p1[k] = ncb[9 * t + k]; p2[k] = ncb[9 * t + 3 + k]; po[k] = ncb[9 * t + 6 + k];
+            p1[k] = W.ncoord[9 * t + k]; p2[k] = W.ncoord[9 * t + 3 + k]; po[k] = W.ncoord[9 * t + 6 + k];
           }
           zero(t, p1, p2, po);
         }
@@ -2591,7 +2573,6 @@
       L.pub_qhead = S.qhead;
       L.pub_qtail = S.qtail;
       L.pub_adopt = adopt ? 1 : 0;
-      L.pub_nnew = nnew;
     }
     ++phase;
 #ifdef LQRO_QHULL_PROFILE
@@ -2706,7 +2687,7 @@
     bool con = false;
     if (f < S.nalloc && (q3_fa(W, L, f) & QF_LIVE)) {
       q3_pl(W, L, f, q);
-      const double* P = W.Pf + 3 * (size_t)W.vv[f].id[0];
+      const double* P = W.Pf + 3 * (size_t)q3_vid0(W, L, f);
       con = fabs(q[0] * (vrel[0] - P[0]) + q[1] * (vrel[1] - P[1]) + q[2] * (vrel[2] - P[2])) <= best + 1e-6 ||
             f == head;
     }
@@ -2717,11 +2698,15 @@
       const int fc = __shfl(f, src);
       double qc[4];
       for (int k = 0; k < 4; k++) qc[k] = __shfl(q[k], src);
-      const int a = W.vv[fc].id[0], b = W.vv[fc].id[1], c = W.vv[fc].id[2];
+      int fcv[3];
+      q3_vid(W, L, fc, fcv);
+      const int a = fcv[0], b = fcv[1], c = fcv[2];
       for (int g = 1 + lane; g < S.nalloc; g += 64) {
         if (!(q3_fa(W, L, g) & QF_LIVE)) continue;
+        int gv[3];
+        q3_vid(W, L, g, gv);
         for (int t = 0; t < 3; t++) {
-          const int id = W.vv[g].id[t];
+          const int id = gv[t];
           if (id == a || id == b || id == c) continue;
           if (q3_distq(qc, W.Pr + 3 * (size_t)id) >= T) sus = true;
         }
@@ -2744,7 +2729,7 @@
       for (int u = 0; u < 4; u++) {
         fs[u] = f0 + 64 * u + lane;
         fa[u] = fs[u] < S.nalloc ? q3_fa(W, L, fs[u]) : 0;
-        v[u] = (fa[u] & QF_LIVE) ? W.vv[fs[u]].id[0] : 0;
+        v[u] = (fa[u] & QF_LIVE) ? q3_vid0(W, L, fs[u]) : 0;
       }
 #pragma unroll
       for (int u = 0; u < 4; u++) {
@@ -2777,7 +2762,7 @@
       if (!(q3_fa(W, L, f) & QF_LIVE)) continue;
       double q[4];
       q3_pl(W, L, f, q);
-      const double* P = W.Pf + 3 * (size_t)W.vv[f].id[0];
+      const double* P = W.Pf + 3 * (size_t)q3_vid0(W, L, f);
       double b;
       const double d0 = qsel_dist(q, P, vrel, &b);
       if (d0 - b > ub) continue;
@@ -2802,8 +2787,7 @@
   const bool merged = (S.status & (QHS_COPLANAR | QHS_NONCONVEX | QHS_FLIPPED | QHS_NARROW | QHS_SINGULAR)) != 0;
   const bool mwin = ok && merged && q3_merge_suspect(W, L, S, lane, vrel, best, head);
   int bv[3] = {0, 0, 0};
-  if (ok)
-    for (int t = 0; t < 3; t++) bv[t] = W.vv[bf].id[t];
+  if (ok) q3_vid(W, L, bf, bv);
   int go = 0;
   if (lane == 0) {
     float* pl = A.planes + (size_t)slot * 8;
@@ -2923,7 +2907,7 @@
     const unsigned long long tjob = __builtin_amdgcn_s_memrealtime();
     const bool spec = A.spec_mark != nullptr && A.spec_mark[slot] >= 2;
     if (threadIdx.x == 0) {
-      L.ph = 0; L.sp_done = 0; L.sp_gdone = 0; L.hctl = 0u; L.hbusy = 0; L.sp_hz = 0; L.pf_done = 0;
+      L.ph = 0; L.sp_done = 0; L.hctl = 0u; L.hbusy = 0; L.sp_hz = 0; L.pf_done = 0;
       L.ectl = 0u; L.edone = 0;
       L.qflags = A.qflags;
 #ifdef LQRO_QHULL_LONGPROF
@@ -2977,8 +2961,6 @@
       Q.qcb = 0; Q.qcn = 0; Q.qf = 0; Q.qp = -1; Q.qk = 0u; Q.qx = Q.qy = Q.qz = 0.0;
       Q.pc_from = -1; Q.pc_pos = -1; Q.pc_end = 0; Q.pc_f = 0; Q.pc_p = -1; Q.pc_k = 0u;
       Q.pc_x = Q.pc_y = Q.pc_z = 0.0;
-      Q.one = 0; Q.rt = -1;
-      for (int k = 0; k < 6; k++) Q.r[k] = 0.0;
       long idle = 0;
       Q3P P;
       for (int k = 0; k < 16; k++) P.t[k] = 0;
@@ -3012,7 +2994,6 @@
           if (lane == 0) L.done_t = __builtin_amdgcn_s_memtime();
 #endif
           if (lane == 0) q3_st_rel_lds(&L.sp_done, p);
-          if (lane == 0) q3_st_rel(&L.sp_gdone, p);
           if (L.qflags & 4) q3_prescan(W, L, lane, ep, ep2, Q);
 #ifdef LQRO_QHULL_PROFILE
           if (lane == 0) { L.done_t2 = __builtin_amdgcn_s_memtime(); L.done_r = __builtin_amdgcn_s_memrealtime(); }
@@ -3172,8 +3153,11 @@
         int rank = 0, nl = 0;
         for (int g = 1; g < S.nalloc; g++)
           if (q3_fa(W, L, g) & QF_LIVE) { nl++; rank += q3_key(W, L, g) < k; }
-        if (rank < A.ext_max)
-          for (int t = 0; t < 3; t++) A.ext_facets[3 * rank + t] = W.vv[f].id[t];
+        if (rank < A.ext_max) {
+          int fv[3];
+          q3_vid(W, L, f, fv);
+          for (int t = 0; t < 3; t++) A.ext_facets[3 * rank + t] = fv[t];
+        }
         if (rank == 0 && nl < A.ext_max) A.ext_facets[3 * nl] = -1;
       }
       hl_sync();
```

New measurement: 59.87 million (median of 6 runs). About the same (+0.6%).
